# CameronDiao/MolCLR

Measured on AMD Instinct MI355X. Metric: contrastive pre-train molecules/sec at batch 512, 1/2/4/8 MI355X; HBM GB/s on scatter_add, higher is better.
Workload: dtype f32; 1 GPU; c2: GIN 5x300 feat 512, batch 512/GPU, 10-50 atom graphs; model=gin 5x300 feat 512, global_batch=512, per_gpu_batch=512, mean_nodes_per_view=15278, mean_edges_per_view=25094, parallelism=dp1, views=one paired encoder pass, per-view BatchNorm statistics, augment=host: pre-built resident batch pairs

## Files before the change

include/molclr.h:

```cpp
#ifndef MOLCLR_H_
#define MOLCLR_H_

#include <stddef.h>
#include <stdint.h>

#ifdef __cplusplus
extern "C" {
#endif

typedef void* molclr_stream_t;

enum {
  MOLCLR_OK = 0,
  MOLCLR_ERR_ARG = -1,
  MOLCLR_ERR_WORKSPACE = -2,
  MOLCLR_ERR_UNSUPPORTED = -3
};

#define MOLCLR_NUM_ATOM_TYPE 119
#define MOLCLR_NUM_CHIRALITY 3
#define MOLCLR_NUM_BOND_TYPE 5
#define MOLCLR_NUM_BOND_DIR 3
#define MOLCLR_SELF_LOOP_BOND_TYPE 4
#define MOLCLR_ECOUNT_STRIDE 8
#define MOLCLR_NUM_ECOMB 15
#define MOLCLR_SELF_LOOP_ECOMB 12
#define MOLCLR_NBR_SLOTS 4
#define MOLCLR_NBR_OVERFLOW 7
#define MOLCLR_NBR_MAX_NODES (1 << 24)
#define MOLCLR_STATUS_ATOM_RANGE 8

#define MOLCLR_ECOMB(ecode) ((int)((ecode) & 7u) * 3 + (int)((ecode) >> 3))

const char* molclr_version(void);
const char* molclr_last_error(void);

size_t molclr_graph_build_workspace_bytes(int64_t num_nodes, int64_t num_edges);
int molclr_graph_build(const int64_t* edge_index, const int64_t* edge_attr,
                       const int64_t* batch, int64_t num_nodes, int64_t num_edges,
                       int64_t num_graphs, int32_t* rowptr, int32_t* col,
                       uint8_t* ecode, int32_t* rowptr_t, int32_t* col_t,
                       uint32_t* nbr, uint32_t* nbr_t,
                       int32_t* ecount, int32_t* graph_ptr, int32_t* status,
                       void* workspace, size_t workspace_bytes, molclr_stream_t stream);

#define MOLCLR_MAX_SEGMENTS 8
typedef struct molclr_graph_segment {
  const int64_t* edge_index;
  const int64_t* edge_attr;
  const int64_t* batch;
  int64_t num_nodes, num_edges, num_graphs;
} molclr_graph_segment;
int molclr_graph_build_multi(int nseg, const molclr_graph_segment* segs, int32_t* rowptr,
                             int32_t* col, uint8_t* ecode, int32_t* rowptr_t, int32_t* col_t,
                             uint32_t* nbr, uint32_t* nbr_t, int32_t* ecount, int32_t* graph_ptr,
                             int32_t* status, void* workspace, size_t workspace_bytes,
                             molclr_stream_t stream);

typedef struct molclr_stage_source {
  const int64_t *x, *edge_index, *edge_attr, *batch;
  int64_t num_nodes, num_edges;
} molclr_stage_source;
typedef struct molclr_graph_staged_segment {
  const int64_t* edge_index;
  const int64_t* edge_attr;
  const int64_t* batch;
  int64_t node_cap, edge_cap, num_graphs;
} molclr_graph_staged_segment;
int molclr_stage_segments(int nseg, const molclr_stage_source* src,
                          const molclr_graph_staged_segment* dst, int64_t* x_all,
                          int64_t num_nodes_cap, int64_t num_edges_cap, int64_t* counts,
                          molclr_stream_t stream);
int molclr_graph_build_dev(int nseg, const molclr_graph_staged_segment* segs, const int64_t* counts,
                           int64_t num_nodes_cap, int64_t num_edges_cap, int32_t* rowptr,
                           int32_t* col, uint8_t* ecode, int32_t* rowptr_t, int32_t* col_t,
                           uint32_t* nbr, uint32_t* nbr_t, int32_t* ecount, int32_t* graph_ptr,
                           int32_t* status, void* workspace, size_t workspace_bytes,
                           molclr_stream_t stream);

size_t molclr_mask_views_workspace_bytes(int64_t batch_size);
int molclr_mask_views(const int64_t* store_x, const int64_t* store_atom_ptr,
                      const int64_t* store_edge_index, const int64_t* store_edge_attr,
                      const int64_t* store_bond_ptr, int64_t store_mols, int64_t store_edges,
                      const int64_t* mol_ids, int64_t batch_size, uint64_t seed, int view,
                      int64_t* x_out, int64_t* edge_index_out, int64_t* edge_attr_out,
                      int64_t* batch_out, int64_t* ptr_out, int64_t num_nodes, int64_t num_edges,
                      int32_t* status, void* workspace, size_t workspace_bytes,
                      molclr_stream_t stream);

enum { MOLCLR_AUG_SUBGRAPH = 0, MOLCLR_AUG_MIX = 1 };
size_t molclr_aug_views_workspace_bytes(int64_t batch_size, int64_t num_nodes, int64_t num_bonds);
int molclr_aug_views_plan(const int64_t* store_atom_ptr, const int64_t* store_edge_index,
                          const int64_t* store_bond_ptr, int64_t store_mols, int64_t store_edges,
                          const int64_t* mol_ids, int64_t batch_size, uint64_t seed, int view,
                          int mode, int64_t num_nodes, int64_t num_bonds, int64_t* ptr_out,
                          int64_t* num_edges_out, int32_t* status, void* workspace,
                          size_t workspace_bytes, molclr_stream_t stream);
size_t molclr_aug_views_big_workspace_bytes(int64_t big_slots, int64_t big_atoms,
                                            int64_t big_bonds);
int molclr_aug_views_plan_big(const int64_t* store_atom_ptr, const int64_t* store_edge_index,
                              const int64_t* store_bond_ptr, int64_t store_mols,
                              int64_t store_edges, const int64_t* mol_ids, int64_t batch_size,
                              uint64_t seed, int view, int mode, int64_t num_nodes,
                              int64_t num_bonds, int64_t* ptr_out, int64_t* num_edges_out,
                              int32_t* status, void* workspace, size_t workspace_bytes,
                              int64_t big_slots, int64_t big_atoms, int64_t big_bonds,
                              void* big_workspace, size_t big_workspace_bytes,
                              molclr_stream_t stream);
int molclr_aug_views_write(const int64_t* store_x, const int64_t* store_atom_ptr,
                           const int64_t* store_edge_index, const int64_t* store_edge_attr,
                           const int64_t* store_bond_ptr, int64_t store_mols, int64_t store_edges,
                           const int64_t* mol_ids, int64_t batch_size, const int64_t* ptr,
                           int64_t num_nodes, int64_t num_bonds, int64_t num_edges, int64_t* x_out,
                           int64_t* edge_index_out, int64_t* edge_attr_out, int64_t* batch_out,
                           const void* workspace, size_t workspace_bytes, molclr_stream_t stream);

int molclr_atom_embed_fwd(const int64_t* x, const float* X1, const float* X2,
                          float* h, int64_t num_nodes, int64_t dim, int64_t n1,
                          int64_t n2, int32_t* status, molclr_stream_t stream);
size_t molclr_atom_embed_bwd_workspace_bytes(int64_t num_nodes, int64_t dim, int64_t n1,
                                             int64_t n2);
int molclr_atom_embed_bwd(const int64_t* x, const float* dh, float* dX1, float* dX2,
                          int64_t num_nodes, int64_t dim, int64_t n1, int64_t n2, int accumulate,
                          void* workspace, size_t workspace_bytes, molclr_stream_t stream);

#define MOLCLR_MAX_LAYERS 16
int molclr_edge_tables_combine(int layers, const float* const* E1s, const float* const* E2s,
                               float* Ec, int64_t dim, molclr_stream_t stream);

int molclr_gine_aggregate_fwd(const float* x, const int32_t* rowptr, const int32_t* col,
                              const uint8_t* ecode, const uint32_t* nbr, const float* Ec,
                              float* out, int64_t num_nodes, int64_t dim,
                              molclr_stream_t stream);
int64_t molclr_rowmax_layout(int64_t D);
size_t molclr_rowmax_bytes(int64_t N, int64_t D);
int molclr_gine_aggregate_fwd_rowmax(const float* x, const int32_t* rowptr, const int32_t* col,
                                     const uint8_t* ecode, const uint32_t* nbr, const float* Ec,
                                     float* out, int64_t N, int64_t D, float* rowparts,
                                     float* slot, molclr_stream_t stream);
int molclr_gine_aggregate_bn_fwd(const float* z, const float* coeffs, int relu, int nseg,
                                 const int64_t* seg_rows, const int64_t* seg_rows_dev,
                                 const int32_t* rowptr, const int32_t* col, const uint8_t* ecode,
                                 const uint32_t* nbr, const float* Ec, float* out, int64_t N,
                                 int64_t D, float* rowparts, float* slot, molclr_stream_t stream);
size_t molclr_gine_aggregate_bwd_workspace_bytes(int64_t num_nodes, int64_t dim);
int molclr_gine_aggregate_bwd(const float* g, const int32_t* rowptr_t, const int32_t* col_t,
                              const uint32_t* nbr_t, const int32_t* ecount, float* dx, float* dE1, float* dE2,
                              int64_t num_nodes, int64_t dim, int accumulate, void* workspace,
                              size_t workspace_bytes, molclr_stream_t stream);
int molclr_gine_aggregate_bwd_impl(const float* g, const int32_t* rowptr_t, const int32_t* col_t,
                                   const uint32_t* nbr_t, const int32_t* ecount, float* dx,
                                   float* dE1, float* dE2, int64_t num_nodes, int64_t dim,
                                   int accumulate, void* workspace, size_t workspace_bytes,
                                   molclr_stream_t stream, int impl);

int molclr_gcn_aggregate_fwd(const float* xw, const int32_t* rowptr, const int32_t* col,
                             const uint8_t* ecode, const uint32_t* nbr, const float* E1,
                             const float* E2,
                             const float* bias, float* out, int64_t num_nodes,
                             int64_t dim, molclr_stream_t stream);
size_t molclr_gcn_aggregate_bwd_workspace_bytes(int64_t num_nodes, int64_t dim);
int molclr_gcn_aggregate_bwd(const float* g, const int32_t* rowptr_t, const int32_t* col_t,
                             const uint32_t* nbr_t, const int32_t* ecount, float* dxw, float* dE1, float* dE2,
                             float* dbias, int64_t num_nodes, int64_t dim, int accumulate,
                             void* workspace, size_t workspace_bytes, molclr_stream_t stream);
int molclr_gcn_aggregate_fwd_bf16(const uint16_t* xw, const int32_t* rowptr, const int32_t* col,
                                  const uint8_t* ecode, const uint32_t* nbr, const float* E1,
                                  const float* E2, const float* bias, uint16_t* out,
                                  int64_t num_nodes, int64_t dim, molclr_stream_t stream);
int molclr_gcn_aggregate_bwd_bf16(const uint16_t* g, const int32_t* rowptr_t,
                                  const int32_t* col_t, const uint32_t* nbr_t,
                                  const int32_t* ecount, uint16_t* dxw, float* dE1, float* dE2,
                                  float* dbias, int64_t num_nodes, int64_t dim, int accumulate,
                                  void* workspace, size_t workspace_bytes,
                                  molclr_stream_t stream);

enum { MOLCLR_EPI_NONE = 0, MOLCLR_EPI_BIAS = 1, MOLCLR_EPI_BIAS_RELU = 2,
       MOLCLR_EPI_RELU_MASK = 3,
       MOLCLR_EPI_ACCUMULATE = 16  };
size_t molclr_gemm_f32_workspace_bytes(int64_t M, int64_t N, int64_t K);
int molclr_gemm_f32(const float* A, const float* B, float* C, int64_t M, int64_t N,
                    int64_t K, int64_t lda, int64_t ldb, int64_t ldc, int a_kmajor,
                    int b_kmajor, int epilogue_flags, const float* bias, const float* aux,
                    int64_t ldaux, void* workspace, size_t workspace_bytes,
                    molclr_stream_t stream);

int molclr_gemm_f32_impl(const float* A, const float* B, float* C, int64_t M, int64_t N,
                         int64_t K, int64_t lda, int64_t ldb, int64_t ldc, int a_kmajor,
                         int b_kmajor, int epilogue_flags, const float* bias, const float* aux,
                         int64_t ldaux, void* workspace, size_t workspace_bytes,
                         molclr_stream_t stream, int impl);

size_t molclr_bplanes_bytes(int64_t N, int64_t K);
int molclr_bplanes_make(const float* B, int64_t N, int64_t K, int64_t ldb, int b_kmajor,
                        uint16_t* planes, molclr_stream_t stream);
int molclr_bplanes_make_batch(int count, const float* const* B, const int64_t* N,
                              const int64_t* K, const int64_t* ldb, const int* b_kmajor,
                              uint16_t* const* planes, molclr_stream_t stream);
int molclr_gemm_f32_bplanes(const float* A, const uint16_t* planes, float* C, int64_t M,
                            int64_t N, int64_t K, int64_t lda, int64_t ldc, int a_kmajor,
                            int epilogue_flags, const float* bias, const float* aux,
                            int64_t ldaux, void* workspace, size_t workspace_bytes,
                            molclr_stream_t stream);
int molclr_gemm_f32_bplanes_tile(const float* A, const uint16_t* planes, float* C, int64_t M,
                                 int64_t N, int64_t K, int64_t lda, int64_t ldc, int a_kmajor,
                                 int epilogue_flags, const float* bias, const float* aux,
                                 int64_t ldaux, void* workspace, size_t workspace_bytes,
                                 molclr_stream_t stream, int tile);

size_t molclr_linear_wgrad_workspace_bytes(int64_t rows, int64_t n_out, int64_t n_in);
int molclr_linear_wgrad(const float* dy, const float* x, float* dW, float* db, int64_t rows,
// ... 134 lines not shown
                                int accumulate, void* workspace, size_t workspace_bytes,
                                molclr_stream_t stream);
int molclr_batchnorm_seg_bwd_frozen(const void* dy, const void* z, const float* gamma,
                                    const float* beta, const float* save_mean,
                                    const float* save_invstd, void* dz, float* dgamma,
                                    float* dbeta, int nseg, const int64_t* seg_rows, int64_t dim,
                                    int dtype, int relu, int accumulate, void* workspace,
                                    size_t workspace_bytes, molclr_stream_t stream);
int molclr_batchnorm_seg_bwd_frozen_dev(const void* dy, const void* z, const float* gamma,
                                        const float* beta, const float* save_mean,
                                        const float* save_invstd, void* dz, float* dgamma,
                                        float* dbeta, int nseg, const int64_t* seg_rows_dev,
                                        int64_t rows_cap, int64_t dim, int dtype, int relu,
                                        int accumulate, float* rowmax, float* slot,
                                        void* workspace, size_t workspace_bytes,
                                        molclr_stream_t stream);
int molclr_batchnorm_seg_bwd_frozen_max(const float* dy, const float* z, const float* gamma,
                                        const float* beta, const float* save_mean,
                                        const float* save_invstd, float* dz, float* dgamma,
                                        float* dbeta, int nseg, const int64_t* seg_rows,
                                        int64_t dim, int relu, int accumulate, float* rowmax,
                                        float* slot, void* workspace, size_t workspace_bytes,
                                        molclr_stream_t stream);

int molclr_segment_pool_fwd(const float* h, const int32_t* graph_ptr, float* out,
                            int64_t num_graphs, int64_t dim, int mode,
                            molclr_stream_t stream);
int molclr_segment_pool_bwd(const float* dout, const int32_t* graph_ptr, float* dh,
                            int64_t num_nodes, int64_t num_graphs, int64_t dim, int mode,
                            molclr_stream_t stream);
int molclr_segment_max_fwd(const void* h, const int32_t* graph_ptr, float* out, int32_t* argmax,
                           int64_t num_graphs, int64_t dim, int dtype, molclr_stream_t stream);
int molclr_segment_max_bwd(const float* dout, const int32_t* argmax, void* dh, int64_t num_nodes,
                           int64_t num_graphs, int64_t dim, int dtype, molclr_stream_t stream);

int molclr_l2norm_fwd(const float* z, float* y, float* norm, int64_t rows, int64_t dim,
                      double eps, molclr_stream_t stream);
int molclr_l2norm_bwd(const float* dy, const float* y, const float* norm, float* dz,
                      int64_t rows, int64_t dim, double eps, molclr_stream_t stream);

int molclr_ntxent_prep(const float* r, float* rhat, float* norm, int64_t n, int64_t C,
                       int cosine, molclr_stream_t stream);
int molclr_ntxent_prep_bwd(const float* drhat, const float* rhat, const float* norm,
                           float* dr, int64_t n, int64_t C, int cosine,
                           molclr_stream_t stream);
int molclr_ntxent_prep_pair(const float* z, float* y, float* rhat, float* n1, float* n2,
                            int64_t batch_local, int64_t C, double eps, int cosine,
                            molclr_stream_t stream);
int molclr_ntxent_prep_pair_bwd(const float* drhat, const float* rhat, const float* n2,
                                const float* y, const float* n1, float* dz, int64_t batch_local,
                                int64_t C, double eps, int cosine, molclr_stream_t stream);
size_t molclr_ntxent_workspace_bytes(int64_t nrows, int64_t ncols, int64_t C);
int molclr_ntxent_fwd(const float* rhat_rows, const int32_t* row_gidx, const float* rhat_cols,
                      int64_t nrows, int64_t ncols, int64_t C, int64_t batch_size,
                      double temperature, float* lse_rows, float* loss_rows,
                      void* workspace, size_t workspace_bytes, molclr_stream_t stream);
int molclr_ntxent_bwd(const float* rhat_rows, const int32_t* row_gidx, const float* rhat_cols,
                      const float* lse_cols, const float* grad_loss, int64_t nrows,
                      int64_t ncols, int64_t C, int64_t batch_size, double temperature,
                      float* drhat_rows, void* workspace, size_t workspace_bytes,
                      molclr_stream_t stream);
size_t molclr_ntxent_sim_bytes(int64_t nrows, int64_t ncols, int64_t C, int impl);
int molclr_ntxent_fwd_impl(const float* rhat_rows, const int32_t* row_gidx,
                           const float* rhat_cols, int64_t nrows, int64_t ncols, int64_t C,
                           int64_t batch_size, double temperature, float* lse_rows,
                           float* loss_rows, float* sim, void* workspace, size_t workspace_bytes,
                           molclr_stream_t stream, int impl);
int molclr_ntxent_bwd_impl(const float* rhat_rows, const int32_t* row_gidx,
                           const float* rhat_cols, const float* lse_cols, const float* grad_loss,
                           int64_t nrows, int64_t ncols, int64_t C, int64_t batch_size,
                           double temperature, const float* sim, float* drhat_rows,
                           void* workspace, size_t workspace_bytes, molclr_stream_t stream,
                           int impl);
int molclr_sum_f32(const float* x, float* out, int64_t n, molclr_stream_t stream);

int molclr_adam_step(float* param, const float* grad, float* exp_avg, float* exp_avg_sq,
                     int64_t n, const float* lr, int32_t* step, double beta1, double beta2,
                     double eps, double weight_decay, molclr_stream_t stream);
int molclr_adam_step_ex(float* param, const float* grad, float* exp_avg, float* exp_avg_sq,
                        int64_t n, const float* lr, int32_t* step, double beta1, double beta2,
                        double eps, double weight_decay, int tick, molclr_stream_t stream);
int molclr_step_tail(int32_t* step, const float* loss_src, float* loss_dst,
                     const int32_t* status_src, int32_t* status_acc, molclr_stream_t stream);

enum {
  MOLCLR_MODE_EVAL = 0,
  MOLCLR_MODE_TRAIN = 1,
  MOLCLR_MODE_FROZEN_BN = 2
};
typedef struct molclr_gin_encoder {
  int32_t num_layer;
  int32_t training;
  int64_t dim;
  int64_t n_atom;
  int64_t n_chiral;
  double momentum, eps;
  const float* x_embedding1;
  const float* x_embedding2;
  const float* mlp0_weight[MOLCLR_MAX_LAYERS];
  const float* mlp0_bias[MOLCLR_MAX_LAYERS];
  const float* mlp2_weight[MOLCLR_MAX_LAYERS];
  const float* mlp2_bias[MOLCLR_MAX_LAYERS];
  const float* edge_embedding1[MOLCLR_MAX_LAYERS];
  const float* edge_embedding2[MOLCLR_MAX_LAYERS];
  const float* bn_weight[MOLCLR_MAX_LAYERS];
  const float* bn_bias[MOLCLR_MAX_LAYERS];
  float* bn_running_mean[MOLCLR_MAX_LAYERS];
  float* bn_running_var[MOLCLR_MAX_LAYERS];
  int64_t* bn_num_batches_tracked[MOLCLR_MAX_LAYERS];
  const uint16_t* mlp0_planes[MOLCLR_MAX_LAYERS];
  const uint16_t* mlp0_planes_t[MOLCLR_MAX_LAYERS];
  const uint16_t* mlp2_planes[MOLCLR_MAX_LAYERS];
  const uint16_t* mlp2_planes_t[MOLCLR_MAX_LAYERS];
  int32_t dtype;
  int32_t fp32_gemm;
  int32_t* status;
  double drop_ratio;
  int64_t* drop_state;
} molclr_gin_encoder;

typedef struct molclr_gin_encoder_grads {
  float* x_embedding1;
  float* x_embedding2;
  float* mlp0_weight[MOLCLR_MAX_LAYERS];
  float* mlp0_bias[MOLCLR_MAX_LAYERS];
  float* mlp2_weight[MOLCLR_MAX_LAYERS];
  float* mlp2_bias[MOLCLR_MAX_LAYERS];
  float* edge_embedding1[MOLCLR_MAX_LAYERS];
  float* edge_embedding2[MOLCLR_MAX_LAYERS];
  float* bn_weight[MOLCLR_MAX_LAYERS];
  float* bn_bias[MOLCLR_MAX_LAYERS];
  void* layer_done[MOLCLR_MAX_LAYERS];
  void* embed_done;
} molclr_gin_encoder_grads;

typedef struct molclr_device_graph {
  int64_t num_nodes, num_edges, num_graphs;
  const int32_t *rowptr, *col, *rowptr_t, *col_t, *ecount, *graph_ptr;
  const uint8_t* ecode;
  const uint32_t *nbr, *nbr_t;
  int32_t num_segments;
  int64_t segment_nodes[MOLCLR_MAX_SEGMENTS];
  const int64_t* segment_nodes_dev;
} molclr_device_graph;

size_t molclr_gin_encoder_arena_bytes(int num_layer, int64_t num_nodes, int64_t dim, int dtype);
size_t molclr_gin_encoder_workspace_bytes(int num_layer, int64_t num_nodes, int64_t dim,
                                          int dtype);
int molclr_gin_encoder_fwd(const molclr_gin_encoder* enc, const int64_t* x,
                           const molclr_device_graph* graph, void* h_out, void* arena,
                           size_t arena_bytes, void* workspace, size_t workspace_bytes,
                           molclr_stream_t stream);
int molclr_gin_encoder_bwd(const molclr_gin_encoder* enc, const molclr_gin_encoder_grads* grads,
                           const int64_t* x, const molclr_device_graph* graph,
                           const void* dh_out, const void* arena, size_t arena_bytes,
                           void* workspace, size_t workspace_bytes, molclr_stream_t stream);

typedef struct molclr_gcn_encoder {
  int32_t num_layer;
  int32_t training;
  int64_t dim;
  int64_t n_atom;
  int64_t n_chiral;
  double momentum, eps;
  const float* x_embedding1;
  const float* x_embedding2;
// ... 244 lines not shown
```

molclr_amd/_lib.py:

```python
from __future__ import annotations

import ctypes
import os
from ctypes import POINTER, c_char_p, c_double, c_int, c_int64, c_size_t, c_uint64, c_void_p
from pathlib import Path

import torch

LIB_PATH = Path(os.environ.get("MOLCLR_LIB", Path(__file__).resolve().parent / "libmolclr_hip.so"))

_P = c_void_p
_I64 = c_int64

SIGNATURES = {
    "molclr_version": (c_char_p, []),
    "molclr_last_error": (c_char_p, []),
    "molclr_graph_build_workspace_bytes": (c_size_t, [_I64, _I64]),
    "molclr_graph_build": (c_int, [_P, _P, _P, _I64, _I64, _I64, _P, _P, _P, _P, _P, _P, _P, _P,
                                   _P, _P, _P, c_size_t, _P]),
    "molclr_graph_build_multi": (c_int, [c_int, _P, _P, _P, _P, _P, _P, _P, _P, _P, _P, _P, _P,
                                         c_size_t, _P]),
    "molclr_stage_segments": (c_int, [c_int, _P, _P, _P, _I64, _I64, _P, _P]),
    "molclr_graph_build_dev": (c_int, [c_int, _P, _P, _I64, _I64, _P, _P, _P, _P, _P, _P, _P, _P,
                                       _P, _P, _P, c_size_t, _P]),
    "molclr_mask_views_workspace_bytes": (c_size_t, [_I64]),
    "molclr_mask_views": (c_int, [_P, _P, _P, _P, _P, _I64, _I64, _P, _I64, c_uint64, c_int, _P, _P,
                                  _P, _P, _P, _I64, _I64, _P, _P, c_size_t, _P]),
    "molclr_atom_embed_fwd": (c_int, [_P, _P, _P, _P, _I64, _I64, _I64, _I64, _P, _P]),
    "molclr_atom_embed_bwd_workspace_bytes": (c_size_t, [_I64, _I64, _I64, _I64]),
    "molclr_atom_embed_bwd": (c_int, [_P, _P, _P, _P, _I64, _I64, _I64, _I64, c_int, _P, c_size_t,
                                      _P]),
    "molclr_edge_tables_combine": (c_int, [c_int, _P, _P, _P, _I64, _P]),
    "molclr_gine_aggregate_fwd": (c_int, [_P, _P, _P, _P, _P, _P, _P, _I64, _I64, _P]),
    "molclr_rowmax_layout": (_I64, [_I64]),
    "molclr_rowmax_bytes": (c_size_t, [_I64, _I64]),
    "molclr_gine_aggregate_fwd_rowmax": (c_int, [_P, _P, _P, _P, _P, _P, _P, _I64, _I64, _P, _P,
                                                 _P]),
    "molclr_gine_aggregate_bn_fwd": (c_int, [_P, _P, c_int, c_int, _P, _P, _P, _P, _P, _P, _P, _P,
                                             _I64, _I64, _P, _P, _P]),
    "molclr_gine_aggregate_bn_fwd_bf16": (c_int, [_P, _P, c_int, c_int, _P, _P, _P, _P, _P, _P, _P,
                                                  _P, _I64, _I64, _P]),
    "molclr_batchnorm_seg_coeffs": (c_int, [_P, _P, _P, _P, _P, _P, _P, _P, _P, c_int, _P, _I64,
                                            c_int, c_double, c_double, c_int, _P, c_size_t, _P]),
    "molclr_batchnorm_seg_coeffs_dev": (c_int, [_P, _P, _P, _P, _P, _P, _P, _P, _P, c_int, _P, _I64,
                                                _I64, c_int, c_double, c_double, c_int, _P,
                                                c_size_t, _P]),
    "molclr_gine_aggregate_bwd_workspace_bytes": (c_size_t, [_I64, _I64]),
    "molclr_gine_aggregate_bwd": (c_int, [_P, _P, _P, _P, _P, _P, _P, _P, _I64, _I64, c_int, _P,
                                          c_size_t, _P]),
    "molclr_gine_aggregate_bwd_impl": (c_int, [_P, _P, _P, _P, _P, _P, _P, _P, _I64, _I64, c_int,
                                               _P, c_size_t, _P, c_int]),
    "molclr_gcn_aggregate_fwd": (c_int, [_P, _P, _P, _P, _P, _P, _P, _P, _P, _I64, _I64, _P]),
    "molclr_gcn_aggregate_bwd_workspace_bytes": (c_size_t, [_I64, _I64]),
    "molclr_gcn_aggregate_bwd": (c_int, [_P, _P, _P, _P, _P, _P, _P, _P, _P, _I64, _I64, c_int,
                                         _P, c_size_t, _P]),
    "molclr_gcn_aggregate_fwd_bf16": (c_int, [_P, _P, _P, _P, _P, _P, _P, _P, _P, _I64, _I64, _P]),
    "molclr_gcn_aggregate_bwd_bf16": (c_int, [_P, _P, _P, _P, _P, _P, _P, _P, _P, _I64, _I64,
                                              c_int, _P, c_size_t, _P]),
    "molclr_gemm_f32_workspace_bytes": (c_size_t, [_I64, _I64, _I64]),
    "molclr_gemm_f32": (c_int, [_P, _P, _P, _I64, _I64, _I64, _I64, _I64, _I64, c_int, c_int, c_int,
                                _P, _P, _I64, _P, c_size_t, _P]),
    "molclr_gemm_f32_impl": (c_int, [_P, _P, _P, _I64, _I64, _I64, _I64, _I64, _I64, c_int, c_int,
                                     c_int, _P, _P, _I64, _P, c_size_t, _P, c_int]),
    "molclr_bplanes_bytes": (c_size_t, [_I64, _I64]),
    "molclr_bplanes_make": (c_int, [_P, _I64, _I64, _I64, c_int, _P, _P]),
    "molclr_bplanes_make_batch": (c_int, [c_int, _P, _P, _P, _P, _P, _P, _P]),
    "molclr_gemm_f32_bplanes": (c_int, [_P, _P, _P, _I64, _I64, _I64, _I64, _I64, c_int, c_int, _P,
                                        _P, _I64, _P, c_size_t, _P]),
    "molclr_gemm_f32_bplanes_tile": (c_int, [_P, _P, _P, _I64, _I64, _I64, _I64, _I64, c_int,
                                             c_int, _P, _P, _I64, _P, c_size_t, _P, c_int]),
    "molclr_linear_wgrad_workspace_bytes": (c_size_t, [_I64, _I64, _I64]),
    "molclr_linear_wgrad": (c_int, [_P, _P, _P, _P, _I64, _I64, _I64, _I64, _I64, c_int, _P, c_size_t,
                                    _P]),
    "molclr_linear_wgrad_groups": (c_int, [_P, _P, _P, _P, _I64, _I64, _I64, _I64, _I64, c_int, _P,
                                           c_size_t, _P, c_int]),
    "molclr_absmax_f32": (c_int, [_P, _I64, _I64, _I64, _P, c_int, _P]),
    "molclr_hplanes_bytes": (c_size_t, [_I64, _I64]),
    "molclr_hplanes_make_batch": (c_int, [c_int, _P, _P, _P, _P, _P, _P, _P]),
    "molclr_absmax_rows_f32": (c_int, [_P, _I64, _I64, _I64, _P, _P, c_int, _P]),
    "molclr_bn_row_parts": (c_int, [_I64]),
    "molclr_batchnorm_seg_bwd_max": (c_int, [_P, _P, _P, _P, _P, _P, _P, _P, _P, c_int, _P, _I64,
                                             c_int, c_int, _P, _P, _P, c_size_t, _P]),
    "molclr_gemm_row_parts": (_I64, [_I64]),
    "molclr_gemm_f32_bplanes_max": (c_int, [_P, _P, _P, _I64, _I64, _I64, _I64, _I64, c_int, _P,
                                            _P, _I64, _P, _P, _P, _P, _P, c_size_t, _P]),
    "molclr_gemm_f32_h3": (c_int, [_P, _P, c_int, _P, _P, _I64, _I64, _I64, _I64, _I64, c_int, _P,
                                   _P, _I64, _P, _P, _P, _P, _P]),
    "molclr_gemm_f32_h3_bits": (c_int, [_P, _P, c_int, _P, _P, _I64, _I64, _I64, _I64, _I64, c_int,
                                        _P, _P, _I64, _P, _P, _P, _P, _P, _P]),
    "molclr_gemm_f32_h3_impl": (c_int, [_P, _P, c_int, _P, _P, _I64, _I64, _I64, _I64, _I64, c_int,
                                        _P, _P, _I64, _P, _P, _P, _P, _P, _P, c_int]),
    "molclr_linear_wgrad_h3_groups": (c_int, [_P, _P, _P, _P, _P, _P, _I64, _I64, _I64, _I64, _I64,
                                              c_int, _P, c_size_t, _P, c_int]),
    "molclr_linear_wgrad_h3": (c_int, [_P, _P, _P, _P, _P, _P, _I64, _I64, _I64, _I64, _I64, c_int,
                                       _P, c_size_t, _P]),
    "molclr_colsum_f32_workspace_bytes": (c_size_t, [_I64, _I64]),
    "molclr_colsum_f32": (c_int, [_P, _P, _I64, _I64, _I64, c_int, _P, c_size_t, _P]),
    "molclr_batchnorm_workspace_bytes": (c_size_t, [_I64, _I64]),
    "molclr_batchnorm_fwd": (c_int, [_P, _P, _P, _P, _P, _P, _P, _P, _P, _I64, _I64, c_double,
                                     c_double, c_int, c_int, _P, c_size_t, _P]),
    "molclr_batchnorm_bwd": (c_int, [_P, _P, _P, _P, _P, _P, _P, _P, _P, _I64, _I64, c_int, c_int,
                                     _P, c_size_t, _P]),
    "molclr_batchnorm_bwd_frozen": (c_int, [_P, _P, _P, _P, _P, _P, _P, _P, _P, _I64, _I64, c_int,
                                            c_int, _P, c_size_t, _P]),
    "molclr_batchnorm_seg_bwd_frozen": (c_int, [_P, _P, _P, _P, _P, _P, _P, _P, _P, c_int, _P, _I64,
                                                c_int, c_int, c_int, _P, c_size_t, _P]),
    "molclr_batchnorm_seg_bwd_frozen_dev": (c_int, [_P, _P, _P, _P, _P, _P, _P, _P, _P, c_int, _P,
                                                    _I64, _I64, c_int, c_int, c_int, _P, _P, _P,
                                                    c_size_t, _P]),
    "molclr_batchnorm_seg_bwd_frozen_max": (c_int, [_P, _P, _P, _P, _P, _P, _P, _P, _P, c_int, _P,
                                                    _I64, c_int, c_int, _P, _P, _P, c_size_t, _P]),
    "molclr_batchnorm_seg_workspace_bytes": (c_size_t, [c_int, _P, _I64]),
    "molclr_batchnorm_seg_fwd": (c_int, [_P, _P, _P, _P, _P, _P, _P, _P, _P, c_int, _P, _I64, c_int,
                                         c_double, c_double, c_int, c_int, _P, c_size_t, _P]),
    "molclr_batchnorm_seg_bwd": (c_int, [_P, _P, _P, _P, _P, _P, _P, _P, _P, c_int, _P, _I64, c_int,
                                         c_int, c_int, _P, c_size_t, _P]),
    "molclr_batchnorm_seg_dev_workspace_bytes": (c_size_t, [c_int, _I64, _I64]),
    "molclr_batchnorm_seg_fwd_dev": (c_int, [_P, _P, _P, _P, _P, _P, _P, _P, _P, c_int, _P, _I64,
                                             _I64, c_int, c_double, c_double, c_int, c_int, _P,
                                             c_size_t, _P]),
    "molclr_batchnorm_seg_bwd_dev": (c_int, [_P, _P, _P, _P, _P, _P, _P, _P, _P, c_int, _P, _I64,
                                             _I64, c_int, c_int, c_int, _P, _P, _P, c_size_t, _P]),
    "molclr_segment_pool_fwd": (c_int, [_P, _P, _P, _I64, _I64, c_int, _P]),
    "molclr_segment_pool_bwd": (c_int, [_P, _P, _P, _I64, _I64, _I64, c_int, _P]),
    "molclr_l2norm_fwd": (c_int, [_P, _P, _P, _I64, _I64, c_double, _P]),
    "molclr_l2norm_bwd": (c_int, [_P, _P, _P, _P, _I64, _I64, c_double, _P]),
    "molclr_ntxent_prep": (c_int, [_P, _P, _P, _I64, _I64, c_int, _P]),
    "molclr_ntxent_prep_bwd": (c_int, [_P, _P, _P, _P, _I64, _I64, c_int, _P]),
    "molclr_ntxent_prep_pair": (c_int, [_P, _P, _P, _P, _P, _I64, _I64, c_double, c_int, _P]),
    "molclr_ntxent_prep_pair_bwd": (c_int, [_P, _P, _P, _P, _P, _P, _I64, _I64, c_double, c_int,
                                            _P]),
    "molclr_ntxent_workspace_bytes": (c_size_t, [_I64, _I64, _I64]),
    "molclr_ntxent_fwd": (c_int, [_P, _P, _P, _I64, _I64, _I64, _I64, c_double, _P, _P, _P,
                                  c_size_t, _P]),
    "molclr_ntxent_bwd": (c_int, [_P, _P, _P, _P, _P, _I64, _I64, _I64, _I64, c_double, _P, _P,
                                  c_size_t, _P]),
    "molclr_ntxent_sim_bytes": (c_size_t, [_I64, _I64, _I64, c_int]),
    "molclr_ntxent_fwd_impl": (c_int, [_P, _P, _P, _I64, _I64, _I64, _I64, c_double, _P, _P,
                                       _P, _P, c_size_t, _P, c_int]),
    "molclr_ntxent_bwd_impl": (c_int, [_P, _P, _P, _P, _P, _I64, _I64, _I64, _I64, c_double, _P,
                                       _P, _P, c_size_t, _P, c_int]),
    "molclr_sum_f32": (c_int, [_P, _P, _I64, _P]),
    "molclr_linear_wgrad_h3_pair_workspace_bytes": (c_size_t, [_I64, _I64, _I64, _I64, _I64]),
    "molclr_linear_wgrad_h3_pair": (c_int, [_P, _P, _P, _P, _P, _P, _I64, _I64, _I64, _I64,
                                            _P, _P, _P, _P, _P, _P, _I64, _I64, _I64, _I64,
                                            _I64, c_int, _P, c_size_t, _P]),
    "molclr_adam_step": (c_int, [_P, _P, _P, _P, _I64, _P, _P, c_double, c_double, c_double,
                                 c_double, _P]),
    "molclr_adam_step_ex": (c_int, [_P, _P, _P, _P, _I64, _P, _P, c_double, c_double, c_double,
                                    c_double, c_int, _P]),
    "molclr_step_tail": (c_int, [_P, _P, _P, _P, _P, _P]),
    "molclr_gin_encoder_arena_bytes": (c_size_t, [c_int, _I64, _I64, c_int]),
    "molclr_gin_encoder_workspace_bytes": (c_size_t, [c_int, _I64, _I64, c_int]),
    "molclr_gin_encoder_fwd": (c_int, [_P, _P, _P, _P, _P, c_size_t, _P, c_size_t, _P]),
    "molclr_gin_encoder_bwd": (c_int, [_P, _P, _P, _P, _P, _P, c_size_t, _P, c_size_t, _P]),
    "molclr_gcn_encoder_arena_bytes": (c_size_t, [c_int, _I64, _I64]),
    "molclr_gcn_encoder_workspace_bytes": (c_size_t, [c_int, _I64, _I64]),
    "molclr_gcn_encoder_arena_bytes_dtype": (c_size_t, [c_int, _I64, _I64, c_int]),
    "molclr_gcn_encoder_workspace_bytes_dtype": (c_size_t, [c_int, _I64, _I64, c_int]),
    "molclr_gcn_encoder_fwd": (c_int, [_P, _P, _P, _P, _P, c_size_t, _P, c_size_t, _P]),
    "molclr_gcn_encoder_bwd": (c_int, [_P, _P, _P, _P, _P, _P, c_size_t, _P, c_size_t, _P]),
    "molclr_dropout_next_key": (c_int, [_P, _P, _P]),
    "molclr_dropout_mask": (c_int, [_P, c_int, c_double, _P, _I64, _I64, _P]),
    "molclr_aug_views_workspace_bytes": (c_size_t, [_I64, _I64, _I64]),
    "molclr_aug_views_plan": (c_int, [_P, _P, _P, _I64, _I64, _P, _I64, ctypes.c_uint64, c_int,
                                      c_int, _I64, _I64, _P, _P, _P, _P, c_size_t, _P]),
    "molclr_aug_views_big_workspace_bytes": (c_size_t, [_I64, _I64, _I64]),
    "molclr_aug_views_plan_big": (c_int, [_P, _P, _P, _I64, _I64, _P, _I64, ctypes.c_uint64,
                                          c_int, c_int, _I64, _I64, _P, _P, _P, _P, c_size_t,
                                          _I64, _I64, _I64, _P, c_size_t, _P]),
    "molclr_aug_views_write": (c_int, [_P, _P, _P, _P, _P, _I64, _I64, _P, _I64, _P, _I64, _I64,
                                       _I64, _P, _P, _P, _P, _P, c_size_t, _P]),
    "molclr_atom_embed_fwd_bf16": (c_int, [_P, _P, _P, _P, _I64, _I64, _I64, _I64, _P, _P]),
    "molclr_atom_embed_bwd_bf16": (c_int, [_P, _P, _P, _P, _I64, _I64, _I64, _I64, c_int, _P,
                                           c_size_t, _P]),
    "molclr_gine_aggregate_fwd_bf16": (c_int, [_P, _P, _P, _P, _P, _P, _P, _I64, _I64, _P]),
    "molclr_gine_aggregate_bwd_bf16": (c_int, [_P, _P, _P, _P, _P, _P, _P, _P, _I64, _I64, c_int,
                                               _P, c_size_t, _P]),
    "molclr_segment_max_fwd": (c_int, [_P, _P, _P, _P, _I64, _I64, c_int, _P]),
    "molclr_segment_max_bwd": (c_int, [_P, _P, _P, _I64, _I64, _I64, c_int, _P]),
    "molclr_segment_pool_fwd_bf16": (c_int, [_P, _P, _P, _I64, _I64, c_int, _P]),
    "molclr_segment_pool_bwd_bf16": (c_int, [_P, _P, _P, _I64, _I64, _I64, c_int, _P]),
    "molclr_gemm_bf16": (c_int, [_P, _P, _P, _I64, _I64, _I64, _I64, _I64, c_int, _P, _P, _I64,
                                 _P]),
    "molclr_gemm_bf16_bits": (c_int, [_P, _P, _P, _I64, _I64, _I64, _I64, _I64, c_int, _P, _P, _P,
                                      _P]),
    "molclr_gemm_bf16_impl": (c_int, [_P, _P, _P, _I64, _I64, _I64, _I64, _I64, c_int, _P, _P,
                                      _I64, _P, c_int]),
    "molclr_linear_wgrad_bf16_workspace_bytes": (c_size_t, [_I64, _I64, _I64]),
    "molclr_linear_wgrad_bf16_impl": (c_int, [_P, _P, _P, _P, _I64, _I64, _I64, _I64, _I64, c_int,
                                              _P, c_size_t, _P, c_int]),
    "molclr_linear_wgrad_bf16": (c_int, [_P, _P, _P, _P, _I64, _I64, _I64, _I64, _I64, c_int, _P,
                                         c_size_t, _P]),
    "molclr_task_head_workspace_bytes": (c_size_t, [_P]),
    "molclr_task_head_fwd": (c_int, [_P, _P, c_size_t, _P]),
    "molclr_task_head_bwd": (c_int, [_P, _P, _P, c_size_t, _P]),
    "molclr_motif_pool_workspace_bytes": (c_size_t, [_I64, _I64, _I64]),
    "molclr_motif_pool_fwd": (c_int, [_P, _P, _P, _P, _P, _P, _I64, _I64, _I64, _I64, _P, _P, _P,
                                      _P]),
    "molclr_motif_pool_bwd": (c_int, [_P, _P, _P, _P, _P, _P, _P, _P, _P, _P, _I64, _I64, _I64, _I64,
                                      _P, _P, _P, _P, c_int, c_int, c_int, _P, c_size_t, _P]),
    "molclr_motif_pool_cap_workspace_bytes": (c_size_t, [_I64, _I64, _I64]),
    "molclr_motif_pool_fwd_cap": (c_int, [_P, _P, _P, _P, _P, _P, _I64, _I64, _I64, _I64, _P, _P,
                                          _P, _P]),
    "molclr_motif_pool_bwd_cap": (c_int, [_P, _P, _P, _P, _P, _P, _P, _P, _P, _P, _I64, _I64, _I64,
                                          _I64, _P, _P, _P, _P, c_int, c_int, c_int, _P, c_size_t,
                                          _P]),
    "molclr_stage_motif": (c_int, [_P, _P, _I64, _I64, _I64, _P, _P, _P, _P, _P, _P]),
    "molclr_stage_task": (c_int, [_P, _P, _P, _I64, _I64, _P, _P, _P, _I64, _I64, c_int, _P]),
    "molclr_task_step_tail": (c_int, [_P, _P, _P, _P, _P, _P, _P]),
    "molclr_eval_tail": (c_int, [_P, _P, _I64, _I64, _I64, _P, _P, _P, _I64, _P, _P, _P, _P, _P]),
    "molclr_collate_task_workspace_bytes": (c_size_t, [_I64]),
    "molclr_collate_task": (c_int, [_P, _P, _P, _P, _P, _I64, _I64, _P, _I64, _P, _I64, c_int, _P,
                                    _P, _P, _P, _P, _P, _I64, _I64, _P, _P, c_size_t, _P]),
    "molclr_stage_task_ids": (c_int, [_P, _P, _P, _P, _P, _I64, _I64, _P, _I64, _P, _I64, c_int,
                                      _I64, _I64, _P, _P, _I64, _I64, _P, _P, _P, _P, c_size_t,
                                      _P]),
    "molclr_motif_items_workspace_bytes": (c_size_t, [_I64]),
    "molclr_motif_items": (c_int, [_P, _P, _I64, _P, _I64, _I64, _P, _P, _P, _P, c_size_t, _P]),
    "molclr_stage_motif_ids_workspace_bytes": (c_size_t, [_I64, _I64]),
    "molclr_stage_motif_ids": (c_int, [_P, _P, _I64, _P, _I64, _I64, _I64, _P, _P, _P, _P, _P, _P,
                                       c_size_t, _P]),
    "molclr_topk_dot_workspace_bytes": (c_size_t, [_I64, _I64, _I64, c_int]),
    "molclr_topk_dot": (c_int, [_P, _I64, _P, _I64, c_int, _I64, _I64, _I64, c_int, _P, _I64, _P,
                                _P, _P, c_size_t, _P]),
    "molclr_ktimer_start": (c_int, [c_int]),
    "molclr_ktimer_read": (c_int, [c_int, _P, _P]),
    "molclr_ktimer_stop": (c_int, []),
}

EPI_NONE, EPI_BIAS, EPI_BIAS_RELU, EPI_RELU_MASK = 0, 1, 2, 3
EPI_ACCUMULATE = 16
NUM_ECOMB = 15
MAX_LAYERS = 16
# ... 165 lines not shown
```

molclr_amd/csrc/aggregate.hip:

```cpp
#include "common.h"

#include <stdlib.h>

namespace {

constexpr int kT = 256;

template <typename St, int U = 1>
__global__ void k_atom_embed_fwd(const int64_t* __restrict__ x, const float4* __restrict__ X1,
                                 const float4* __restrict__ X2, typename St::T* __restrict__ h,
                                 int64_t N, int d4, int64_t n1, int64_t n2,
                                 int32_t* __restrict__ status) {
  int64_t t = (int64_t)blockIdx.x * blockDim.x + threadIdx.x;
  if (t >= N * d4 / U) return;
  const int64_t u0 = t * U;
  int64_t i = N * d4 < (1ll << 32) ? (int64_t)((uint32_t)u0 / (uint32_t)d4) : u0 / d4;
  int c = (int)(u0 - i * d4);
  const int64_t a = x[2 * i], b = x[2 * i + 1];
  float4 v[U];
  if (a < 0 || a >= n1 || b < 0 || b >= n2) {
    const float q = __builtin_nanf("");
#pragma unroll
    for (int j = 0; j < U; ++j) v[j] = make_float4(q, q, q, q);
    if (c == 0 && status != nullptr) atomicOr(status, MOLCLR_STATUS_ATOM_RANGE);
  } else {
#pragma unroll
    for (int j = 0; j < U; ++j) v[j] = f4add(X1[a * d4 + c + j], X2[b * d4 + c + j]);
  }
  if constexpr (U == 2) St::st2(h, t, v[0], v[1]);
  else St::st(h, t, v[0]);
}

constexpr int kEmbBlock = 256;
constexpr int kEmbChunk = 128;

__device__ __forceinline__ int emb_key(const int64_t* __restrict__ x, int64_t item, int64_t N,
                                       int64_t n1, int64_t n2) {
  if (item < N) {
    const int64_t a = x[2 * item];
    return (int)(a < 0 ? 0 : (a >= n1 ? n1 - 1 : a));
  }
  const int64_t b = x[2 * (item - N) + 1];
  return (int)(n1 + (b < 0 ? 0 : (b >= n2 ? n2 - 1 : b)));
}

__global__ __launch_bounds__(kEmbBlock) void k_emb_hist(const int64_t* __restrict__ x, int64_t N,
                                                        int64_t n1, int64_t n2,
                                                        int32_t* __restrict__ hist) {
  extern __shared__ int32_t h[];
  const int nk = (int)(n1 + n2);
  for (int k = threadIdx.x; k < nk; k += kEmbBlock) h[k] = 0;
  __syncthreads();
  const int64_t item = (int64_t)blockIdx.x * kEmbBlock + threadIdx.x;
  if (item < 2 * N) atomicAdd(&h[emb_key(x, item, N, n1, n2)], 1);
  __syncthreads();
  for (int k = threadIdx.x; k < nk; k += kEmbBlock) hist[(int64_t)k * gridDim.x + blockIdx.x] = h[k];
}

__global__ __launch_bounds__(64) void k_emb_keyscan(int32_t* __restrict__ hist, int nblk,
                                                    int32_t* __restrict__ total) {
  const int64_t k = blockIdx.x;
  const int lane = threadIdx.x;
  int32_t* row = hist + k * nblk;
  int32_t carry = 0;
  for (int base = 0; base < nblk; base += 64) {
    const int b = base + lane;
    const int32_t v = b < nblk ? row[b] : 0;
    int32_t incl = v;
#pragma unroll
    for (int o = 1; o < 64; o <<= 1) {
      const int32_t u = __shfl_up(incl, o, 64);
      if (lane >= o) incl += u;
    }
    if (b < nblk) row[b] = carry + incl - v;
    carry += __shfl(incl, 63, 64);
  }
  if (lane == 0) total[k] = carry;
}

__global__ __launch_bounds__(1024) void k_emb_plan(const int32_t* __restrict__ total, int nk,
                                                   int32_t* __restrict__ kstart,
                                                   int32_t* __restrict__ cbeg,
                                                   int32_t* __restrict__ cend,
                                                   int32_t* __restrict__ kchunk0,
                                                   int32_t* __restrict__ nchunks, int max_chunks) {
  __shared__ int32_t tot[1024], ks[1025], kc[1025];
  const int t = threadIdx.x;
  tot[t] = t < nk ? total[t] : 0;
  __syncthreads();
  if (t == 0) {
    int32_t run = 0, ch = 0;
    for (int k = 0; k < nk; ++k) {
      ks[k] = run;
      kc[k] = ch;
      run += tot[k];
      ch += (tot[k] + kEmbChunk - 1) / kEmbChunk;
    }
    ks[nk] = run;
    kc[nk] = ch;
    *nchunks = ch;
  }
  __syncthreads();
  for (int k = t; k <= nk; k += 1024) {
    kstart[k] = ks[k];
    kchunk0[k] = kc[k];
  }
  const int nch = kc[nk];
  for (int c = t; c < max_chunks; c += 1024) {
    if (c >= nch) break;
    int lo = 0, hi = nk - 1;
    while (lo < hi) {
      const int mid = (lo + hi + 1) >> 1;
      if (kc[mid] <= c) lo = mid;
// ... 49 lines not shown
  for (; i + 4 <= end; i += 4) {
    float4 v[4];
#pragma unroll
    for (int u = 0; u < 4; ++u) v[u] = St::ld(dh, (int64_t)perm[i + u] * d4 + c);
#pragma unroll
    for (int u = 0; u < 4; ++u) acc = f4add(acc, v[u]);
  }
  for (; i < end; ++i) acc = f4add(acc, St::ld(dh, (int64_t)perm[i] * d4 + c));
  double* o = csum + ch * 4 * d4 + 4 * c;
  o[0] = acc.x;
  o[1] = acc.y;
  o[2] = acc.z;
  o[3] = acc.w;
}

constexpr int kEmbFinW = 8;
__global__ __launch_bounds__(64 * kEmbFinW) void k_emb_finish(
    const double* __restrict__ csum, const int32_t* __restrict__ kchunk0, int64_t n1, int64_t n2,
    int64_t D, float* __restrict__ dX1, float* __restrict__ dX2, int accumulate) {
  __shared__ double red[kEmbFinW][64];
  const int lane = threadIdx.x & 63, w = threadIdx.x >> 6;
  const int64_t k = blockIdx.x;
  const int64_t col = (int64_t)blockIdx.y * 64 + lane;
  double acc = 0.0;
  if (col < D) {
    int32_t ch = kchunk0[k] + w;
    const int32_t ce = kchunk0[k + 1];
    for (; ch + 7 * kEmbFinW < ce; ch += 8 * kEmbFinW) {
      double v[8];
#pragma unroll
      for (int u = 0; u < 8; ++u) v[u] = csum[(int64_t)(ch + u * kEmbFinW) * D + col];
#pragma unroll
      for (int u = 0; u < 8; ++u) acc += v[u];
    }
    for (; ch < ce; ch += kEmbFinW) acc += csum[(int64_t)ch * D + col];
  }
  red[w][lane] = acc;
  __syncthreads();
  if (w != 0 || col >= D) return;
  double t = red[0][lane];
#pragma unroll
  for (int q = 1; q < kEmbFinW; ++q) t += red[q][lane];
  float* o = k < n1 ? dX1 + k * D + col : dX2 + (k - n1) * D + col;
  *o = accumulate ? *o + (float)t : (float)t;
}

__global__ __launch_bounds__(1024) void k_reduce_partials_split(
    const double* __restrict__ partial, int64_t P, int64_t rows, int64_t D, int64_t split,
    float* __restrict__ outA, float* __restrict__ outB, int accumulate) {
  constexpr int EL = 16, LANES = 64;
  __shared__ double red[LANES][EL];
  const int cl = threadIdx.x % EL, rl = threadIdx.x / EL;
  const int64_t t = (int64_t)blockIdx.x * EL + cl;
  const int64_t n = rows * D;
  double a0 = 0.0, a1 = 0.0, a2 = 0.0, a3 = 0.0;
  if (t < n) {
    int64_t p = rl;
    for (; p + 3 * LANES < P; p += 4 * LANES) {
      a0 += partial[p * n + t];
      a1 += partial[(p + LANES) * n + t];
      a2 += partial[(p + 2 * LANES) * n + t];
      a3 += partial[(p + 3 * LANES) * n + t];
    }
    for (; p < P; p += LANES) a0 += partial[p * n + t];
  }
  double acc = (a0 + a1) + (a2 + a3);
  red[rl][cl] = acc;
  __syncthreads();
#pragma unroll
  for (int stride = LANES / 2; stride > 0; stride >>= 1) {
    if (rl < stride) red[rl][cl] = acc = acc + red[rl + stride][cl];
    __syncthreads();
  }
  if (rl != 0 || t >= n) return;
  int64_t r = t / D;
  float* o = r < split ? (outA ? outA + t : nullptr) : (outB ? outB + (t - split * D) : nullptr);
  if (o) *o = accumulate ? *o + (float)acc : (float)acc;
}

struct TablePtrs {
  const float* e1[MOLCLR_MAX_LAYERS];
  const float* e2[MOLCLR_MAX_LAYERS];
};
__global__ void k_edge_tables_combine(TablePtrs p, float* __restrict__ Ec, int layers, int64_t D,
                                      float* __restrict__ zero, int64_t n_zero) {
  const int64_t per = (int64_t)MOLCLR_NUM_ECOMB * D;
  int64_t t = (int64_t)blockIdx.x * blockDim.x + threadIdx.x;
  if (t < n_zero) zero[t] = 0.f;
  if (t >= layers * per) return;
  const int l = (int)(t / per);
  const int64_t rc = t - l * per;
  const int r = (int)(rc / D);
  const int64_t c = rc - (int64_t)r * D;
  Ec[t] = p.e1[l][(r / 3) * D + c] + p.e2[l][(r % 3) * D + c];
}

__device__ __forceinline__ uint32_t nbr_degree(uint32_t w0) { return w0 >> 29; }
__device__ __forceinline__ int32_t nbr_node(uint32_t w) { return (int32_t)(w & 0xFFFFFFu); }
__device__ __forceinline__ int nbr_ecomb(uint32_t w) { return (int)((w >> 24) & 15u); }

__device__ __forceinline__ float4 gine_msg(const float4* __restrict__ x, const float4* __restrict__ Ec,
                                           uint32_t w, int d4, int c) {
  return f4add(x[(int64_t)nbr_node(w) * d4 + c], Ec[nbr_ecomb(w) * d4 + c]);
}

struct NoSrcArgs {};
template <typename DR>
struct BnSrcArgsT {
  const float4* scale;
  const float4* shift;
  int relu;
  Segs sg;
  DR drop;
};
typedef BnSrcArgsT<NoDrop> BnSrcArgs;

template <typename St, typename DR>
__device__ __forceinline__ float4 bn_src_unit(float4 v, float4 sc, float4 sh, bool relu,
                                              const Drop<DR>& drop, int64_t j, int c4) {
  float4 o = make_float4(bn_apply1(v.x, sc.x, sh.x), bn_apply1(v.y, sc.y, sh.y),
                         bn_apply1(v.z, sc.z, sh.z), bn_apply1(v.w, sc.w, sh.w));
  if (relu) o = make_float4(fmaxf(o.x, 0.f), fmaxf(o.y, 0.f), fmaxf(o.z, 0.f), fmaxf(o.w, 0.f));
  if constexpr (DR::kOn) o = drop(o, j, c4);
  if constexpr (St::kBytes == 2) {
    const uint32_t lo = f32x2_to_bf16x2(o.x, o.y), hi = f32x2_to_bf16x2(o.z, o.w);
    o = make_float4(bf16_to_f32(lo & 0xFFFFu), bf16_to_f32(lo >> 16), bf16_to_f32(hi & 0xFFFFu),
                    bf16_to_f32(hi >> 16));
  }
  return o;
}

template <typename St, typename SA>
struct AggSrc {
  __device__ __forceinline__ AggSrc(const SA&, int64_t, int, int) {}
  __device__ __forceinline__ float4 operator()(const typename St::T* __restrict__ x, int64_t unit,
                                               int64_t) const {
    return St::ld(x, unit);
  }
};
template <typename St, typename DR>
struct AggSrc<St, BnSrcArgsT<DR>> {
  float4 sc, sh;
  bool relu, pad;
  int c;
  Drop<DR> drop;
  __device__ __forceinline__ AggSrc(const BnSrcArgsT<DR>& a, int64_t i, int c_, int d4)
      : c(c_), drop(a.drop) {
    const int s = seg_of_row(a.sg, i);
    pad = s < 0;
    relu = a.relu != 0;
    sc = pad ? f4zero() : a.scale[s * d4 + c];
    sh = pad ? f4zero() : a.shift[s * d4 + c];
  }
  __device__ __forceinline__ float4 operator()(const typename St::T* __restrict__ x, int64_t unit,
                                               int64_t j) const {
    if (pad) return f4zero();
    return bn_src_unit<St, DR>(St::ld(x, unit), sc, sh, relu, drop, j, c);
  }
};

template <typename St, bool NT = false, typename SA = NoSrcArgs>
__device__ __forceinline__ float4 gine_agg_elem(
    const typename St::T* __restrict__ x, const int32_t* __restrict__ rowptr,
    const int32_t* __restrict__ col, const uint8_t* __restrict__ ecode,
    const uint4* __restrict__ nbr, const float4* __restrict__ Ec, typename St::T* __restrict__ out,
    int64_t t, int64_t i, int c, int d4, const SA& sa) {
  const AggSrc<St, SA> src(sa, i, c, d4);
  auto X = [&](int64_t j) { return src(x, j * d4 + c, j); };
  auto msg = [&](uint32_t w) {
    return f4add(X((int64_t)nbr_node(w)), Ec[nbr_ecomb(w) * d4 + c]);
  };
  const uint4 s = nbr[i];
  const float4 self = src(x, t, i);
  const float4 es = Ec[MOLCLR_SELF_LOOP_ECOMB * d4 + c];
  const uint32_t deg = nbr_degree(s.x);
  float4 acc = f4zero();
  if (deg <= MOLCLR_NBR_SLOTS) {
// ... 558 lines not shown

template <typename St>
int emb_bwd(const int64_t* x, const typename St::T* dh, float* dX1, float* dX2, int64_t N,
            int64_t D, int64_t n1, int64_t n2, int accumulate, void* workspace,
            size_t workspace_bytes, hipStream_t s) {
  const int64_t nk = n1 + n2;
  const EmbWs e = emb_ws(workspace, workspace_bytes, N, D, n1, n2);
  const int64_t d4 = D / 4;
  if (N > 0) {
    hipLaunchKernelGGL(k_emb_hist, dim3((unsigned)e.nblk), dim3(kEmbBlock), nk * sizeof(int32_t), s,
                       x, N, n1, n2, e.hist);
  } else {
    (void)molclr::zero_async(e.hist, (size_t)e.nblk * nk * sizeof(int32_t), s);
  }
  hipLaunchKernelGGL(k_emb_keyscan, dim3((unsigned)nk), dim3(64), 0, s, e.hist, (int)e.nblk,
                     e.total);
  hipLaunchKernelGGL(k_emb_plan, dim3(1), dim3(1024), 0, s, static_cast<const int32_t*>(e.total),
                     (int)nk, e.kstart, e.cbeg, e.cend, e.kchunk0, e.nchunks, (int)e.max_chunks);
  if (N > 0) {
    hipLaunchKernelGGL(k_emb_scatter, dim3((unsigned)e.nblk), dim3(kEmbBlock), 0, s, x, N, n1, n2,
                       static_cast<const int32_t*>(e.hist), static_cast<const int32_t*>(e.kstart),
                       e.perm);
    hipLaunchKernelGGL(k_emb_chunk_sum<St>, dim3((unsigned)e.max_chunks,
                                                 (unsigned)molclr::ceil_div(d4, 64)),
                       dim3(64), 0, s, dh, static_cast<const int32_t*>(e.perm),
                       static_cast<const int32_t*>(e.cbeg), static_cast<const int32_t*>(e.cend),
                       static_cast<const int32_t*>(e.nchunks), d4, e.csum);
  }
  hipLaunchKernelGGL(k_emb_finish, dim3((unsigned)nk, (unsigned)molclr::ceil_div(D, 64)),
                     dim3(64 * kEmbFinW), 0, s,
                     static_cast<const double*>(e.csum), static_cast<const int32_t*>(e.kchunk0), n1,
                     n2, D, dX1, dX2, accumulate);
  MOLCLR_LAUNCHED();
  return MOLCLR_OK;
}
}

MOLCLR_API size_t molclr_atom_embed_bwd_workspace_bytes(int64_t N, int64_t D, int64_t n1,
                                                        int64_t n2) {
  const int64_t nk = n1 + n2;
  const int64_t nblk = molclr::ceil_div(2 * N > 0 ? 2 * N : 1, (int64_t)kEmbBlock);
  const int64_t max_chunks = molclr::ceil_div(2 * N, (int64_t)kEmbChunk) + nk;
  return (size_t)(nblk * nk + nk + 2 * (nk + 1) + 2 * max_chunks + 1 + 2 * N) * sizeof(int32_t) +
         (size_t)max_chunks * D * sizeof(double) + 10 * 256;
}

MOLCLR_API int molclr_atom_embed_bwd(const int64_t* x, const float* dh, float* dX1, float* dX2,
                                     int64_t N, int64_t D, int64_t n1, int64_t n2, int accumulate,
                                     void* workspace, size_t workspace_bytes,
                                     molclr_stream_t stream) {
  MOLCLR_REQUIRE(D > 0 && D % 4 == 0 && n1 > 0 && n2 > 0 && N >= 0,
                 "atom_embed_bwd: bad sizes (dim a multiple of 4)");
  MOLCLR_REQUIRE(n1 + n2 <= 1024, "atom_embed_bwd: tables too large");
  MOLCLR_REQUIRE(2 * N < (1ll << 31), "atom_embed_bwd: too many nodes");
  MOLCLR_REQUIRE_WS(workspace_bytes, molclr_atom_embed_bwd_workspace_bytes(N, D, n1, n2));
  return emb_bwd<StF32>(x, dh, dX1, dX2, N, D, n1, n2, accumulate, workspace, workspace_bytes,
                        molclr::as_stream(stream));
}

MOLCLR_API int molclr_edge_tables_combine(int layers, const float* const* E1s,
                                          const float* const* E2s, float* Ec, int64_t D,
                                          molclr_stream_t stream) {
  return molclr::edge_tables_combine_zero(layers, E1s, E2s, Ec, D, nullptr, 0, stream);
}

int molclr::edge_tables_combine_zero(int layers, const float* const* E1s, const float* const* E2s,
                                     float* Ec, int64_t D, float* zero, int64_t n_zero,
                                     molclr_stream_t stream) {
  MOLCLR_REQUIRE(layers >= 0 && layers <= MOLCLR_MAX_LAYERS && D > 0,
                 "edge_tables_combine: %d layers (max %d), dim %lld", layers, MOLCLR_MAX_LAYERS,
                 (long long)D);
  if (layers == 0) return MOLCLR_OK;
  MOLCLR_REQUIRE(E1s && E2s && Ec, "edge_tables_combine: null pointer");
  TablePtrs p{};
  for (int l = 0; l < layers; ++l) {
    MOLCLR_REQUIRE(E1s[l] && E2s[l], "edge_tables_combine: null table of layer %d", l);
    p.e1[l] = E1s[l];
    p.e2[l] = E2s[l];
  }
  const int64_t n = (int64_t)layers * MOLCLR_NUM_ECOMB * D;
  const int64_t work = n > n_zero ? n : n_zero;
  hipLaunchKernelGGL(k_edge_tables_combine, dim3(molclr::ceil_div(work, kT)), dim3(kT), 0,
                     molclr::as_stream(stream), p, Ec, layers, D, zero, n_zero);
  MOLCLR_LAUNCHED();
  return MOLCLR_OK;
}

static bool agg_nt() {
  static const bool on = molclr::env_is("MOLCLR_AGG_NT", '1');
  return on;
}

MOLCLR_API int molclr_gine_aggregate_fwd(const float* x, const int32_t* rowptr,
                                         const int32_t* col, const uint8_t* ecode,
                                         const uint32_t* nbr, const float* Ec, float* out,
                                         int64_t N, int64_t D, molclr_stream_t stream) {
  MOLCLR_REQUIRE(D > 0 && D % 4 == 0, "gine_aggregate_fwd: dim %lld must be a multiple of 4",
                 (long long)D);
  if (N == 0) return MOLCLR_OK;
  MOLCLR_REQUIRE(x && rowptr && nbr && Ec && out, "gine_aggregate_fwd: null pointer");
  int d4 = (int)(D / 4);
  molclr::launch_timed(molclr::kTimeGineAgg, agg_nt() ? k_gine_agg_fwd<StF32, false, true>
                                                      : k_gine_agg_fwd<StF32, false, false>,
                       dim3(molclr::ceil_div(N * d4, kT)), dim3(kT), 0, molclr::as_stream(stream),
                       x, rowptr, col, ecode, (const uint4*)nbr, (const float4*)Ec, out, N, d4,
                       nullptr, 0, nullptr, NoSrcArgs{});
  MOLCLR_LAUNCHED();
  return MOLCLR_OK;
}

MOLCLR_API int64_t molclr_rowmax_layout(int64_t D) {
  const int64_t d4 = D / 4;
  return d4 >= 64 ? -d4 : (int64_t)molclr_bn_row_parts(D);
}
MOLCLR_API size_t molclr_rowmax_bytes(int64_t N, int64_t D) {
  const int64_t code = molclr_rowmax_layout(D);
  return code < 0 ? (size_t)((N * (D / 4) + 63) / 64) * 2 * sizeof(float)
                  : (size_t)code * N * sizeof(float);
}

MOLCLR_API int molclr_gine_aggregate_fwd_rowmax(const float* x, const int32_t* rowptr,
                                                const int32_t* col, const uint8_t* ecode,
                                                const uint32_t* nbr, const float* Ec, float* out,
                                                int64_t N, int64_t D, float* rowparts, float* slot,
                                                molclr_stream_t stream) {
  MOLCLR_REQUIRE(D > 0 && D % 4 == 0, "gine_aggregate_fwd_rowmax: dim %lld must be a multiple of 4",
                 (long long)D);
  MOLCLR_REQUIRE(N < (1ll << 31), "gine_aggregate_fwd_rowmax: too many rows");
  if (N == 0) return MOLCLR_OK;
  MOLCLR_REQUIRE(x && rowptr && nbr && Ec && out && rowparts,
                 "gine_aggregate_fwd_rowmax: null pointer");
  const int d4 = (int)(D / 4);
  static_assert(kT % 64 == 0, "row parts follow the waves");
  molclr::launch_timed(molclr::kTimeGineAgg, agg_nt() ? k_gine_agg_fwd<StF32, true, true>
                                                      : k_gine_agg_fwd<StF32, true, false>,
                       dim3(molclr::ceil_div(N * d4, kT)), dim3(kT), 0, molclr::as_stream(stream),
                       x, rowptr, col, ecode, (const uint4*)nbr, (const float4*)Ec, out, N, d4,
                       rowparts, (int)molclr_rowmax_layout(D), slot, NoSrcArgs{});
  MOLCLR_LAUNCHED();
  return MOLCLR_OK;
}

MOLCLR_API size_t molclr_gine_aggregate_bwd_workspace_bytes(int64_t N, int64_t D) {
  if (!molclr::band_dim_ok(D)) return 0;
  return (size_t)ecount_parts(N, molclr::make_band(D).band) * 8 * D * sizeof(double) + 256;
}

static bool agg_bwd_fused() {
  static const bool on = !molclr::env_is("MOLCLR_AGG_BWD_FUSED", '0');
  return on;
}

MOLCLR_API int molclr_gine_aggregate_bwd_impl(const float* g, const int32_t* rowptr_t,
                                              const int32_t* col_t, const uint32_t* nbr_t,
                                              const int32_t* ecount, float* dx, float* dE1,
                                              float* dE2, int64_t N, int64_t D, int accumulate,
                                              void* workspace, size_t workspace_bytes,
                                              molclr_stream_t stream, int impl) {
  MOLCLR_REQUIRE(molclr::band_dim_ok(D),
                 "gine_aggregate_bwd: dim %lld must be a multiple of 4 in [4, %lld]", (long long)D,
                 (long long)molclr::kBandMaxDim);
  MOLCLR_REQUIRE(impl >= -1 && impl <= 1, "gine_aggregate_bwd: impl %d (-1, 0 or 1)", impl);
  hipStream_t s = molclr::as_stream(stream);
  int d4 = (int)(D / 4);
  const bool fusable = dx && (dE1 || dE2) && N > 0;
  if (fusable && (impl < 0 ? agg_bwd_fused() : impl == 1)) {
// ... 382 lines not shown
```

molclr_amd/csrc/encoder.hip:

```cpp
#include "common.h"

#include <stdlib.h>

namespace {

bool agg_bn() {
  static const bool on = !molclr::env_is("MOLCLR_AGG_BN", '0');
  return on;
}

struct ArenaLayout {
  size_t agg[MOLCLR_MAX_LAYERS], a1[MOLCLR_MAX_LAYERS], z[MOLCLR_MAX_LAYERS],
      h[MOLCLR_MAX_LAYERS], mean[MOLCLR_MAX_LAYERS], invstd[MOLCLR_MAX_LAYERS],
      coef[MOLCLR_MAX_LAYERS];
  size_t bits[MOLCLR_MAX_LAYERS];
  size_t h0, ec, smax, bmax, dropkey, total;
  ArenaLayout(int L, int64_t N, int64_t D, size_t es) {
    size_t used = 0;
    auto off = [&](size_t bytes) {
      const size_t o = used;
      used += (bytes + 255) / 256 * 256;
      return o;
    };
    for (int l = 0; l < L; ++l) {
      agg[l] = off(N * D * es);
      a1[l] = off(N * 2 * D * es);
      z[l] = off(N * D * es);
      h[l] = agg_bn() ? 0 : off(N * D * es);
      mean[l] = off(MOLCLR_MAX_SEGMENTS * D * sizeof(float));
      invstd[l] = off(MOLCLR_MAX_SEGMENTS * D * sizeof(float));
      coef[l] = off(2 * MOLCLR_MAX_SEGMENTS * D * sizeof(float));
      bits[l] = off((size_t)N * ((2 * D + 31) / 32) * sizeof(uint32_t));
    }
    h0 = off(N * D * es);
    ec = off((size_t)L * MOLCLR_NUM_ECOMB * D * sizeof(float));
    smax = off((size_t)MOLCLR_MAX_LAYERS * 2 * kMaxSlotFloats * sizeof(float));
    bmax = off((size_t)MOLCLR_MAX_LAYERS * 2 * kMaxSlotFloats * sizeof(float));
    dropkey = off(2 * sizeof(int64_t));
    total = used;
  }
};

size_t elem_bytes(int dtype) { return dtype == MOLCLR_DTYPE_BF16 ? 2 : 4; }

size_t kernels_ws(int64_t N, int64_t D) {
  size_t m = 0;
  auto mx = [&](size_t v) { m = v > m ? v : m; };
  mx(molclr_gemm_f32_workspace_bytes(2 * D, D, N));
  mx(molclr_gemm_f32_workspace_bytes(D, 2 * D, N));
  mx(molclr_gemm_f32_workspace_bytes(N, 2 * D, D));
  mx(molclr_gemm_f32_workspace_bytes(N, D, 2 * D));
  mx(molclr_colsum_f32_workspace_bytes(N, 2 * D));
  mx(molclr_linear_wgrad_workspace_bytes(N, D, 2 * D));
  mx(molclr_linear_wgrad_workspace_bytes(N, 2 * D, D));
  if (N >= 1024 && D % 4 == 0) mx(molclr_linear_wgrad_h3_pair_workspace_bytes(N, D, 2 * D, 2 * D, D));
  mx(molclr_linear_wgrad_bf16_workspace_bytes(N, D, 2 * D));
  mx(molclr_linear_wgrad_bf16_workspace_bytes(N, 2 * D, D));
  mx(molclr_batchnorm_ws_bound(N, D));
  mx(molclr_gine_aggregate_bwd_workspace_bytes(N, D));
  mx(molclr_atom_embed_bwd_workspace_bytes(N, D, MOLCLR_NUM_ATOM_TYPE, MOLCLR_NUM_CHIRALITY));
  return m;
}

size_t scratch_bytes(int64_t N, int64_t D, size_t es) { return ((size_t)N * D * 3 + (size_t)N * 2 * D) * es; }

template <typename E>
int bn_batch_stats(const E* e) { return e->training == MOLCLR_MODE_TRAIN; }

int check_drop(const char* who, double drop_ratio, const int64_t* drop_state, int training) {
  MOLCLR_REQUIRE(training == MOLCLR_MODE_EVAL || training == MOLCLR_MODE_TRAIN ||
                     training == MOLCLR_MODE_FROZEN_BN,
                 "%s: training %d (MOLCLR_MODE_*)", who, training);
  MOLCLR_REQUIRE(drop_ratio >= 0.0 && drop_ratio < 1.0, "%s: drop_ratio %g outside [0, 1)", who,
                 drop_ratio);
  MOLCLR_REQUIRE(!(training && drop_ratio > 0.0) || drop_state,
                 "%s: training with dropout needs drop_state", who);
  return MOLCLR_OK;
}

int check_encoder(const molclr_gin_encoder* e, const molclr_device_graph* g) {
  MOLCLR_REQUIRE(e && g, "gin_encoder: null encoder / graph");
  MOLCLR_TRY_RC(check_drop("gin_encoder", e->drop_ratio, e->drop_state, e->training));
  MOLCLR_REQUIRE(e->num_layer >= 1 && e->num_layer <= MOLCLR_MAX_LAYERS,
                 "gin_encoder: num_layer %d", e->num_layer);
  MOLCLR_REQUIRE(e->dim > 0 && e->dim % 4 == 0, "gin_encoder: dim %lld", (long long)e->dim);
  MOLCLR_REQUIRE(e->dtype == MOLCLR_DTYPE_F32 || (e->dtype == MOLCLR_DTYPE_BF16 && e->dim % 8 == 0),
                 "gin_encoder: dtype %d (bf16 needs dim %% 8 == 0)", e->dtype);
  MOLCLR_REQUIRE(e->n_atom == MOLCLR_NUM_ATOM_TYPE && e->n_chiral == MOLCLR_NUM_CHIRALITY,
                 "gin_encoder: embedding tables must be [%d,D] and [%d,D]",
                 MOLCLR_NUM_ATOM_TYPE, MOLCLR_NUM_CHIRALITY);
// ... 82 lines not shown
    if (!on) return nullptr;
    cur = make_drop_args(key, p, l);
    return &cur;
  }
};
int open_drop(const CallDrop& d, int64_t* state, molclr_stream_t stream) {
  if (!d.on) return MOLCLR_OK;
  return molclr_dropout_next_key(state, const_cast<int64_t*>(d.key), stream);
}

#define MOLCLR_TRY(expr)      \
  do {                        \
    int rc_ = (expr);         \
    if (rc_) return rc_;      \
  } while (0)

int record_done(void* ev, molclr_stream_t stream) {
  if (ev && hipEventRecord(static_cast<hipEvent_t>(ev), molclr::as_stream(stream)) != hipSuccess) {
    molclr::set_error("encoder_bwd: hipEventRecord failed");
    return MOLCLR_ERR_ARG;
  }
  return MOLCLR_OK;
}

}

MOLCLR_API size_t molclr_gin_encoder_arena_bytes(int L, int64_t N, int64_t D, int dtype) {
  if (L < 1 || L > MOLCLR_MAX_LAYERS) return 0;
  return ArenaLayout(L, N, D, elem_bytes(dtype)).total;
}

constexpr size_t kSlotBytes = MOLCLR_MAX_LAYERS * 2 * kMaxSlotFloats * sizeof(float);
size_t rowmax_first_bytes(int64_t N, int64_t D) {
  const size_t dz = (size_t)molclr_bn_row_parts(D) * N * sizeof(float);
  const size_t agg = molclr_rowmax_bytes(N, D);
  return molclr::align_up(dz > agg ? dz : agg, 256);
}
size_t rowmax_bytes(int64_t N, int64_t D) {
  return molclr::align_up(
      rowmax_first_bytes(N, D) + (size_t)molclr_gemm_row_parts(2 * D) * N * sizeof(float), 256);
}

MOLCLR_API size_t molclr_gin_encoder_workspace_bytes(int L, int64_t N, int64_t D, int dtype) {
  (void)L;
  return molclr::align_up(scratch_bytes(N, D, elem_bytes(dtype)), 256) + kSlotBytes +
         rowmax_bytes(N, D) + kernels_ws(N, D) + 256;
}

MOLCLR_API int molclr_gin_encoder_fwd(const molclr_gin_encoder* e, const int64_t* x,
                                      const molclr_device_graph* g, void* h_out, void* arena,
                                      size_t arena_bytes, void* workspace, size_t workspace_bytes,
                                      molclr_stream_t stream) {
  MOLCLR_TRY(check_encoder(e, g));
  const int L = e->num_layer;
  const int64_t N = g->num_nodes, D = e->dim;
  if (N == 0) return MOLCLR_OK;
  SegRows seg;
  MOLCLR_TRY(graph_segments(g, &g->num_nodes, seg));
  MOLCLR_REQUIRE(x && h_out && arena, "gin_encoder_fwd: null pointer");
  const bool bf = e->dtype == MOLCLR_DTYPE_BF16;
  const size_t es = elem_bytes(e->dtype);
  const ArenaLayout lay(L, N, D, es);
  MOLCLR_REQUIRE_WS(arena_bytes, lay.total);
  MOLCLR_REQUIRE_WS(workspace_bytes, molclr_gin_encoder_workspace_bytes(L, N, D, e->dtype));
  char* A = (char*)arena;
  auto F = [&](size_t off) { return (float*)(A + off); };
  auto H = [&](size_t off) { return (uint16_t*)(A + off); };
  float* ragg = (float*)((char*)workspace + molclr::align_up(scratch_bytes(N, D, es), 256) +
                         kSlotBytes);
  float* ra1 = (float*)((char*)ragg + rowmax_first_bytes(N, D));
  void* kws = (char*)ragg + rowmax_bytes(N, D);
  const size_t kws_bytes = kernels_ws(N, D);
  const bool h3 = !bf && e->fp32_gemm != 0;
  const bool h3f = h3 && (e->fp32_gemm & 2);
  float* fmax = F(lay.smax);

  const bool fused = agg_bn();
  CallDrop drop(e->training, e->drop_ratio, A + lay.dropkey);
  MOLCLR_TRY(open_drop(drop, e->drop_state, stream));
  void* h = A + lay.h0;
  if (bf)
    MOLCLR_TRY(molclr_atom_embed_fwd_bf16(x, e->x_embedding1, e->x_embedding2, (uint16_t*)h, N, D,
                                          e->n_atom, e->n_chiral, e->status, stream));
  else
    MOLCLR_TRY(molclr_atom_embed_fwd(x, e->x_embedding1, e->x_embedding2, (float*)h, N, D,
                                     e->n_atom, e->n_chiral, e->status, stream));
  float* Ec = F(lay.ec);
  const int64_t nz = h3 ? (int64_t)(lay.bmax - lay.smax) / 4 + (int64_t)L * 2 * kMaxSlotFloats : 0;
  MOLCLR_TRY(molclr::edge_tables_combine_zero(L, e->edge_embedding1, e->edge_embedding2, Ec, D,
                                              h3 ? fmax : nullptr, nz, stream));
  for (int l = 0; l < L; ++l) {
    const bool last = l == L - 1;
    const bool bn_src = fused && l > 0;
    const bool bn_next = fused && !last;
    void* y = last ? h_out : bn_next ? nullptr : A + lay.h[l];
    const float* Ecl = Ec + (size_t)l * MOLCLR_NUM_ECOMB * D;
    const void* zp = bn_src ? A + lay.z[l - 1] : nullptr;
    const float* cp = bn_src ? F(lay.coef[l - 1]) : nullptr;
    if (bf) {
      uint16_t *agg = H(lay.agg[l]), *a1 = H(lay.a1[l]), *z = H(lay.z[l]);
      if (bn_src && drop.on)
        MOLCLR_TRY(molclr::gine_aggregate_bn_fwd_drop(zp, cp, 1, seg.n, seg.rows, seg.dev,
                                                      g->rowptr, g->col, g->ecode, g->nbr, Ecl,
                                                      agg, N, D, MOLCLR_DTYPE_BF16, nullptr,
                                                      nullptr, *drop.at(l - 1),
                                                      molclr::as_stream(stream)));
      else if (bn_src)
        MOLCLR_TRY(molclr_gine_aggregate_bn_fwd_bf16((const uint16_t*)zp, cp, 1, seg.n, seg.rows,
                                                     seg.dev, g->rowptr, g->col, g->ecode, g->nbr,
                                                     Ecl, agg, N, D, stream));
      else
        MOLCLR_TRY(molclr_gine_aggregate_fwd_bf16((const uint16_t*)h, g->rowptr, g->col, g->ecode,
                                                  g->nbr, Ecl, agg, N, D, stream));
      if (D % 64 == 0)
        MOLCLR_TRY(molclr_gemm_bf16_bits(agg, e->mlp0_planes[l], a1, N, 2 * D, D, D, 2 * D,
                                         MOLCLR_EPI_BIAS_RELU, e->mlp0_bias[l],
                                         (uint32_t*)(A + lay.bits[l]), nullptr, stream));
      else
        MOLCLR_TRY(molclr_gemm_bf16(agg, e->mlp0_planes[l], a1, N, 2 * D, D, D, 2 * D,
                                    MOLCLR_EPI_BIAS_RELU, e->mlp0_bias[l], nullptr, 0, stream));
      MOLCLR_TRY(molclr_gemm_bf16(a1, e->mlp2_planes[l], z, N, D, 2 * D, 2 * D, D,
                                  MOLCLR_EPI_BIAS, e->mlp2_bias[l], nullptr, 0, stream));
      if (bn_next)
        MOLCLR_TRY(seg_bn_coeffs(seg, z, e->bn_weight[l], e->bn_bias[l], e->bn_running_mean[l],
                                 e->bn_running_var[l], e->bn_num_batches_tracked[l],
                                 F(lay.mean[l]), F(lay.invstd[l]), F(lay.coef[l]), D,
                                 MOLCLR_DTYPE_BF16, e->momentum, e->eps, bn_batch_stats(e), kws,
                                 kws_bytes, stream));
      else
        MOLCLR_TRY(seg_bn_fwd(seg, z, e->bn_weight[l], e->bn_bias[l], e->bn_running_mean[l],
                              e->bn_running_var[l], e->bn_num_batches_tracked[l], y,
                              F(lay.mean[l]), F(lay.invstd[l]), D, MOLCLR_DTYPE_BF16, e->momentum,
                              e->eps, bn_batch_stats(e), last ? 0 : 1, drop.at(l), kws, kws_bytes,
                              stream));
    } else {
      float *agg = F(lay.agg[l]), *a1 = F(lay.a1[l]), *z = F(lay.z[l]);
      float* sl = fmax + 2 * l * kMaxSlotFloats;
      if (bn_src && drop.on)
        MOLCLR_TRY(molclr::gine_aggregate_bn_fwd_drop(zp, cp, 1, seg.n, seg.rows, seg.dev,
                                                      g->rowptr, g->col, g->ecode, g->nbr, Ecl,
                                                      agg, N, D, MOLCLR_DTYPE_F32,
                                                      h3f ? ragg : nullptr, nullptr,
                                                      *drop.at(l - 1), molclr::as_stream(stream)));
      else if (bn_src)
        MOLCLR_TRY(molclr_gine_aggregate_bn_fwd((const float*)zp, cp, 1, seg.n, seg.rows, seg.dev,
                                                g->rowptr, g->col, g->ecode, g->nbr, Ecl, agg, N,
                                                D, h3f ? ragg : nullptr, nullptr, stream));
      else if (h3f)
        MOLCLR_TRY(molclr_gine_aggregate_fwd_rowmax((const float*)h, g->rowptr, g->col, g->ecode,
                                                    g->nbr, Ecl, agg, N, D, ragg, nullptr,
                                                    stream));
      else
        MOLCLR_TRY(molclr_gine_aggregate_fwd((const float*)h, g->rowptr, g->col, g->ecode, g->nbr,
                                             Ecl, agg, N, D, stream));
      if (h3f) {
        const uint16_t* p0 = e->mlp0_planes[l];
        const uint16_t* p2 = e->mlp2_planes[l];
        MOLCLR_TRY(molclr_gemm_f32_h3_bits(agg, ragg, (int)molclr_rowmax_layout(D), p0, a1, N,
                                           2 * D, D, D, 2 * D, MOLCLR_EPI_BIAS_RELU,
                                           e->mlp0_bias[l], nullptr, 0, nullptr,
                                           sl + kMaxSlotFloats, ra1, sl,
                                           (uint32_t*)(A + lay.bits[l]), stream));
        MOLCLR_TRY(molclr_gemm_f32_h3(a1, ra1, (int)molclr_gemm_row_parts(2 * D), p2, z, N, D,
                                      2 * D, 2 * D, D, MOLCLR_EPI_BIAS, e->mlp2_bias[l], nullptr, 0,
                                      nullptr,
                                      nullptr, nullptr, nullptr, stream));
      } else {
        if (h3)
          MOLCLR_TRY(molclr_gemm_f32_bplanes_max(agg, e->mlp0_planes[l], a1, N, 2 * D, D, D, 2 * D,
                                                 MOLCLR_EPI_BIAS_RELU, e->mlp0_bias[l], nullptr, 0,
                                                 fmax + 2 * l * kMaxSlotFloats,
                                                 fmax + (2 * l + 1) * kMaxSlotFloats, nullptr,
                                                 (uint32_t*)(A + lay.bits[l]), kws, kws_bytes,
// ... 434 lines not shown
```

molclr_amd/csrc/graph.hip:

```cpp
#include "common.h"
#include "stage.h"

namespace {

constexpr int kScanThreads = 1024;

struct GSegs {
  int n;
  const int64_t* ei[MOLCLR_MAX_SEGMENTS];
  const int64_t* ea[MOLCLR_MAX_SEGMENTS];
  const int64_t* batch[MOLCLR_MAX_SEGMENTS];
  int64_t n0[MOLCLR_MAX_SEGMENTS + 1], e0[MOLCLR_MAX_SEGMENTS + 1], g0[MOLCLR_MAX_SEGMENTS + 1];
  int64_t eld[MOLCLR_MAX_SEGMENTS];
  const int64_t* dcount;
};

__device__ __forceinline__ int gseg(const int64_t* off, int n, int64_t k) {
  int s = 0;
  while (s + 1 < n && k >= off[s + 1]) ++s;
  return s;
}

__device__ __forceinline__ int64_t gcount(const GSegs& sg, int which, int s) {
  if (sg.dcount) return sg.dcount[which * sg.n + s];
  return which ? sg.e0[s + 1] - sg.e0[s] : sg.n0[s + 1] - sg.n0[s];
}
__device__ __forceinline__ int64_t gbase(const GSegs& sg, int which, int s) {
  if (!sg.dcount) return which ? sg.e0[s] : sg.n0[s];
  int64_t b = 0;
  for (int q = 0; q < s; ++q) b += sg.dcount[which * sg.n + q];
  return b;
}
struct GLoc {
  int s;
  int64_t base, cnt;
};
__device__ __forceinline__ GLoc glocate(const GSegs& sg, int which, int64_t k) {
  int64_t b = 0;
  for (int s = 0; s < sg.n; ++s) {
    const int64_t c = gcount(sg, which, s);
    if (k < b + c) return {s, b, c};
    b += c;
  }
  return {-1, b, 0};
}

__global__ void k_graph_init(int32_t* __restrict__ ecount, int32_t* __restrict__ counters,
                             int64_t n_counters, int64_t N, int32_t* __restrict__ status) {
  int64_t t = (int64_t)blockIdx.x * blockDim.x + threadIdx.x;
  if (t == 0) *status = 0;
  if (t < n_counters) counters[t] = 0;
  if (t < N * MOLCLR_ECOUNT_STRIDE) {
    int j = (int)(t % MOLCLR_ECOUNT_STRIDE);
    ecount[t] = (j == MOLCLR_SELF_LOOP_BOND_TYPE || j == 5) ? 1 : 0;
  }
}

__device__ void graph_ptr_item(const GSegs& sg, int64_t t, int64_t N, int64_t G,
                               int32_t* __restrict__ graph_ptr, int32_t* __restrict__ status);

__global__ void k_graph_count(GSegs sg, int64_t E, int32_t* __restrict__ src32,
                              int32_t* __restrict__ dst32, uint8_t* __restrict__ code8,
                              int32_t* __restrict__ indeg, int32_t* __restrict__ outdeg,
                              int32_t* __restrict__ ecount, int32_t* __restrict__ status, int64_t N,
                              int64_t G, int32_t* __restrict__ graph_ptr) {
  int64_t k = (int64_t)blockIdx.x * blockDim.x + threadIdx.x;
  if (blockIdx.y == 1) {
    if (k < (N > G + 1 ? N : G + 1)) graph_ptr_item(sg, k, N, G, graph_ptr, status);
    return;
  }
  if (k >= E) return;
  const GLoc le = glocate(sg, 1, k);
  if (le.s < 0) return;
  const int g = le.s;
  const int64_t kk = k - le.base, Eg = le.cnt;
  const int64_t Ng = gcount(sg, 0, g), nb = gbase(sg, 0, g);
  const int64_t* ei = sg.ei[g];
  const int64_t* ea = sg.ea[g];
  int64_t s = ei[kk], d = ei[(sg.dcount ? sg.eld[g] : Eg) + kk];
  int64_t bt = ea[2 * kk], bd = ea[2 * kk + 1];
  int bad = 0;
  if (s < 0 || s >= Ng || d < 0 || d >= Ng) {
    bad |= 1;
    s = s < 0 ? 0 : (s >= Ng ? Ng - 1 : s);
    d = d < 0 ? 0 : (d >= Ng ? Ng - 1 : d);
  }
  if (bt < 0 || bt >= MOLCLR_NUM_BOND_TYPE || bd < 0 || bd >= MOLCLR_NUM_BOND_DIR) {
    bad |= 2;
    bt = bt < 0 ? 0 : (bt >= MOLCLR_NUM_BOND_TYPE ? MOLCLR_NUM_BOND_TYPE - 1 : bt);
    bd = bd < 0 ? 0 : (bd >= MOLCLR_NUM_BOND_DIR ? MOLCLR_NUM_BOND_DIR - 1 : bd);
  }
  if (bad) atomicOr(status, bad);
  s += nb;
  d += nb;
  src32[k] = (int32_t)s;
  dst32[k] = (int32_t)d;
  code8[k] = (uint8_t)(bt | (bd << 3));
  atomicAdd(&indeg[d], 1);
  atomicAdd(&outdeg[s], 1);
  atomicAdd(&ecount[d * MOLCLR_ECOUNT_STRIDE + bt], 1);
  atomicAdd(&ecount[d * MOLCLR_ECOUNT_STRIDE + 5 + bd], 1);
}

constexpr int kScanPer = 8;
__global__ __launch_bounds__(kScanThreads) void k_scan2(const int32_t* __restrict__ degA,
                                                        int32_t* __restrict__ ptrA,
                                                        const int32_t* __restrict__ degB,
                                                        int32_t* __restrict__ ptrB, int64_t n) {
  constexpr int TILE = kScanPer * kScanThreads;
  const int32_t* deg = blockIdx.y == 0 ? degA : degB;
  int32_t* ptr = blockIdx.y == 0 ? ptrA : ptrB;
  __shared__ int32_t tile[TILE];
  __shared__ int32_t wsum[kScanThreads / 64];
  const int tid = threadIdx.x, lane = tid & 63, wid = tid >> 6;
  const int64_t base = (int64_t)blockIdx.x * TILE;
  int32_t nx[kScanPer];
#pragma unroll
  for (int c = 0; c < kScanPer; ++c) {
    const int64_t idx = base + (int64_t)c * kScanThreads + tid;
    nx[c] = idx < n ? deg[idx] : 0;
  }
  int32_t pre = 0;
  for (int64_t i0 = tid; i0 < base; i0 += (int64_t)kScanPer * kScanThreads) {
    int32_t q[kScanPer];
#pragma unroll
    for (int c = 0; c < kScanPer; ++c) {
      const int64_t i = i0 + (int64_t)c * kScanThreads;
      q[c] = i < base ? deg[i] : 0;
    }
#pragma unroll
    for (int c = 0; c < kScanPer; ++c) pre += q[c];
  }
#pragma unroll
  for (int o = 32; o > 0; o >>= 1) pre += __shfl_xor(pre, o, 64);
  if (lane == 0) wsum[wid] = pre;
#pragma unroll
  for (int c = 0; c < kScanPer; ++c) tile[c * kScanThreads + tid] = nx[c];
  __syncthreads();
  int32_t carry = 0;
#pragma unroll
  for (int w = 0; w < kScanThreads / 64; ++w) carry += wsum[w];
  int32_t v[kScanPer], x = 0;
#pragma unroll
  for (int j = 0; j < kScanPer; ++j) {
    v[j] = tile[kScanPer * tid + j];
    x += v[j];
  }
  const int32_t own = x;
#pragma unroll
  for (int o = 1; o < 64; o <<= 1) {
    const int32_t u = __shfl_up(x, o, 64);
    if (lane >= o) x += u;
  }
  __syncthreads();
  if (lane == 63) wsum[wid] = x;
  __syncthreads();
  if (wid == 0) {
    int32_t w = lane < kScanThreads / 64 ? wsum[lane] : 0;
#pragma unroll
    for (int o = 1; o < 64; o <<= 1) {
      const int32_t u = __shfl_up(w, o, 64);
      if (lane >= o) w += u;
    }
    if (lane < kScanThreads / 64) wsum[lane] = w;
  }
  __syncthreads();
  int32_t run = carry + (wid > 0 ? wsum[wid - 1] : 0) + x - own;
#pragma unroll
  for (int j = 0; j < kScanPer; ++j) {
    const int64_t idx = base + (int64_t)kScanPer * tid + j;
    if (idx < n) ptr[idx] = run;
    run += v[j];
  }
  if (tid == 0 && base + TILE >= n) ptr[n] = carry + wsum[kScanThreads / 64 - 1];
}

__global__ void k_graph_fill(GSegs sg, const int32_t* __restrict__ src32,
                             const int32_t* __restrict__ dst32, int64_t E,
                             const int32_t* __restrict__ rowptr,
                             const int32_t* __restrict__ rowptr_t, int32_t* __restrict__ cur,
                             int32_t* __restrict__ cur_t, int32_t* __restrict__ perm,
                             int32_t* __restrict__ perm_t) {
  int64_t k = (int64_t)blockIdx.x * blockDim.x + threadIdx.x;
  if (k >= E || (sg.dcount && k >= gbase(sg, 1, sg.n))) return;
  int32_t s = src32[k], d = dst32[k];
  perm[rowptr[d] + atomicAdd(&cur[d], 1)] = (int32_t)k;
  perm_t[rowptr_t[s] + atomicAdd(&cur_t[s], 1)] = (int32_t)k;
}

__global__ void k_graph_rows(int64_t N, const int32_t* __restrict__ src32,
                             const int32_t* __restrict__ dst32, const uint8_t* __restrict__ code8,
                             const int32_t* __restrict__ rowptr, const int32_t* __restrict__ rowptr_t,
                             int32_t* __restrict__ perm, int32_t* __restrict__ perm_t,
                             int32_t* __restrict__ col, uint8_t* __restrict__ ecode,
                             int32_t* __restrict__ col_t, uint4* __restrict__ nbr,
                             uint4* __restrict__ nbr_t) {
  int64_t t = (int64_t)blockIdx.x * blockDim.x + threadIdx.x;
  if (t >= 2 * N) return;
  bool csc = t >= N;
  int64_t i = csc ? t - N : t;
  const int32_t* ptr = csc ? rowptr_t : rowptr;
  int32_t* p = csc ? perm_t : perm;
  int32_t beg = ptr[i], end = ptr[i + 1];
  for (int32_t a = beg + 1; a < end; ++a) {
    int32_t key = p[a];
    int32_t b = a - 1;
    while (b >= beg && p[b] > key) {
      p[b + 1] = p[b];
      --b;
    }
    p[b + 1] = key;
  }
  uint32_t slot[MOLCLR_NBR_SLOTS] = {0u, 0u, 0u, 0u};
  if (!csc) {
    for (int32_t a = beg; a < end; ++a) {
      int32_t k = p[a];
      col[a] = src32[k];
      ecode[a] = code8[k];
      if (a - beg < MOLCLR_NBR_SLOTS)
        slot[a - beg] = (uint32_t)src32[k] | ((uint32_t)MOLCLR_ECOMB(code8[k]) << 24);
    }
  } else {
    for (int32_t a = beg; a < end; ++a) {
      col_t[a] = dst32[p[a]];
      if (a - beg < MOLCLR_NBR_SLOTS) slot[a - beg] = (uint32_t)dst32[p[a]];
    }
  }
  const int32_t deg = end - beg;
  slot[0] |= (uint32_t)(deg > MOLCLR_NBR_SLOTS ? MOLCLR_NBR_OVERFLOW : deg) << 29;
  (csc ? nbr_t : nbr)[i] = make_uint4(slot[0], slot[1], slot[2], slot[3]);
}

__device__ void graph_ptr_item(const GSegs& sg, int64_t t, int64_t N, int64_t G,
                               int32_t* __restrict__ graph_ptr, int32_t* __restrict__ status) {
  if (t < N) {
    const GLoc ln = glocate(sg, 0, t);
    if (ln.s >= 0) {
      const int g = ln.s;
      const int64_t* batch = sg.batch[g];
      const int64_t i = t - ln.base, Gg = sg.g0[g + 1] - sg.g0[g];
      const int64_t b = batch[i];
      if (b < 0 || b >= Gg || (i > 0 && batch[i - 1] > b)) atomicOr(status, 4);
    }
  }
  if (t <= G) {
    if (t == G) {
      graph_ptr[t] = (int32_t)gbase(sg, 0, sg.n);
    } else {
      const int g = gseg(sg.g0, sg.n, t);
      const int64_t* batch = sg.batch[g];
      const int64_t want = t - sg.g0[g];
      int64_t lo = 0, hi = gcount(sg, 0, g);
      while (lo < hi) {
        int64_t mid = (lo + hi) >> 1;
        if (batch[mid] < want) lo = mid + 1;
        else hi = mid;
      }
      graph_ptr[t] = (int32_t)(gbase(sg, 0, g) + lo);
    }
  }
}

int build_launch(const GSegs& sg, int64_t N, int64_t E, int64_t G, int32_t* rowptr, int32_t* col,
                 uint8_t* ecode, int32_t* rowptr_t, int32_t* col_t, uint32_t* nbr, uint32_t* nbr_t,
                 int32_t* ecount, int32_t* graph_ptr, int32_t* status, void* workspace,
                 size_t workspace_bytes, molclr_stream_t stream) {
  MOLCLR_REQUIRE(rowptr && rowptr_t && ecount && graph_ptr && status && (N == 0 || (nbr && nbr_t)),
                 "graph_build: null output");
  MOLCLR_REQUIRE(E == 0 || (col && ecode && col_t), "graph_build: null edge buffer");
  MOLCLR_REQUIRE_WS(workspace_bytes, molclr_graph_build_workspace_bytes(N, E));
  hipStream_t s = molclr::as_stream(stream);
  molclr::Workspace w(workspace, workspace_bytes);
  int32_t* src32 = w.take<int32_t>(E);
  int32_t* dst32 = w.take<int32_t>(E);
  uint8_t* code8 = w.take<uint8_t>(E);
  int32_t* counters = w.take<int32_t>(4 * N);
  int32_t* indeg = counters;
  int32_t* outdeg = counters + N;
  int32_t* cur = counters + 2 * N;
  int32_t* cur_t = counters + 3 * N;
  int32_t* perm = w.take<int32_t>(E);
  int32_t* perm_t = w.take<int32_t>(E);

  const int T = 256;
  int64_t n_init = 8 * N > 4 * N ? 8 * N : 4 * N;
  if (n_init < 1) n_init = 1;
  hipLaunchKernelGGL(k_graph_init, dim3(molclr::ceil_div(n_init, T)), dim3(T), 0, s, ecount,
                     counters, 4 * N, N, status);
  const int64_t n_ptr = N > G + 1 ? N : G + 1;
  const int64_t bx = molclr::ceil_div(E > n_ptr ? E : n_ptr, T);
  hipLaunchKernelGGL(k_graph_count, dim3((unsigned)bx, 2), dim3(T), 0, s, sg, E, src32, dst32,
                     code8, indeg, outdeg, ecount, status, N, G, graph_ptr);
  hipLaunchKernelGGL(k_scan2,
                     dim3((unsigned)(N > 0 ? molclr::ceil_div(N, kScanPer * kScanThreads) : 1), 2),
                     dim3(kScanThreads), 0, s, indeg, rowptr, outdeg, rowptr_t, N);
  if (E > 0) {
    hipLaunchKernelGGL(k_graph_fill, dim3(molclr::ceil_div(E, T)), dim3(T), 0, s, sg, src32, dst32,
                       E, rowptr, rowptr_t, cur, cur_t, perm, perm_t);
  }
  if (N > 0) {
    hipLaunchKernelGGL(k_graph_rows, dim3(molclr::ceil_div(2 * N, T)), dim3(T), 0, s, N, src32,
                       dst32, code8, rowptr, rowptr_t, perm, perm_t, col, ecode, col_t,
                       (uint4*)nbr, (uint4*)nbr_t);
  }
  MOLCLR_LAUNCHED();
  return MOLCLR_OK;
}

}

MOLCLR_API size_t molclr_graph_build_workspace_bytes(int64_t N, int64_t E) {
  molclr::Workspace w(nullptr, 0);
  w.take<int32_t>(E);
  w.take<int32_t>(E);
  w.take<uint8_t>(E);
  w.take<int32_t>(4 * N);
  w.take<int32_t>(E);
  w.take<int32_t>(E);
  return w.used + 256;
}

MOLCLR_API int molclr_graph_build_multi(int nseg, const molclr_graph_segment* segs,
                                        int32_t* rowptr, int32_t* col, uint8_t* ecode,
                                        int32_t* rowptr_t, int32_t* col_t, uint32_t* nbr,
                                        uint32_t* nbr_t, int32_t* ecount, int32_t* graph_ptr,
                                        int32_t* status, void* workspace, size_t workspace_bytes,
                                        molclr_stream_t stream) {
  MOLCLR_REQUIRE(nseg >= 1 && nseg <= MOLCLR_MAX_SEGMENTS && segs,
                 "graph_build: %d segments (1..%d)", nseg, MOLCLR_MAX_SEGMENTS);
  GSegs sg{};
  sg.n = nseg;
  for (int g = 0; g < nseg; ++g) {
    const molclr_graph_segment& q = segs[g];
    MOLCLR_REQUIRE(q.num_nodes >= 0 && q.num_edges >= 0 && q.num_graphs >= 0,
                   "graph_build: negative size in segment %d", g);
    sg.ei[g] = q.edge_index;
    sg.ea[g] = q.edge_attr;
    sg.batch[g] = q.batch;
    sg.n0[g + 1] = sg.n0[g] + q.num_nodes;
    sg.e0[g + 1] = sg.e0[g] + q.num_edges;
    sg.g0[g + 1] = sg.g0[g] + q.num_graphs;
  }
  for (int g = nseg; g < MOLCLR_MAX_SEGMENTS; ++g) {
    sg.n0[g + 1] = sg.n0[nseg];
    sg.e0[g + 1] = sg.e0[nseg];
    sg.g0[g + 1] = sg.g0[nseg];
  }
  const int64_t N = sg.n0[nseg], E = sg.e0[nseg], G = sg.g0[nseg];
  MOLCLR_REQUIRE(N <= MOLCLR_NBR_MAX_NODES && E < (int64_t)1 << 31,
                 "graph_build: %lld nodes exceed the neighbour-slot limit %d (or E > int32)",
                 (long long)N, MOLCLR_NBR_MAX_NODES);
  for (int g = 0; g < nseg; ++g) {
    MOLCLR_REQUIRE(segs[g].num_edges == 0 || (segs[g].edge_index && segs[g].edge_attr),
                   "graph_build: null edge input in segment %d", g);
    MOLCLR_REQUIRE(segs[g].num_nodes == 0 || segs[g].batch, "graph_build: null batch in segment %d",
                   g);
  }
  return build_launch(sg, N, E, G, rowptr, col, ecode, rowptr_t, col_t, nbr, nbr_t, ecount,
                      graph_ptr, status, workspace, workspace_bytes, stream);
}

MOLCLR_API int molclr_graph_build(const int64_t* edge_index, const int64_t* edge_attr,
                                  const int64_t* batch, int64_t N, int64_t E, int64_t G,
                                  int32_t* rowptr, int32_t* col, uint8_t* ecode,
                                  int32_t* rowptr_t, int32_t* col_t, uint32_t* nbr,
                                  uint32_t* nbr_t, int32_t* ecount, int32_t* graph_ptr,
                                  int32_t* status, void* workspace,
                                  size_t workspace_bytes, molclr_stream_t stream) {
  const molclr_graph_segment seg{edge_index, edge_attr, batch, N, E, G};
  return molclr_graph_build_multi(1, &seg, rowptr, col, ecode, rowptr_t, col_t, nbr, nbr_t, ecount,
                                  graph_ptr, status, workspace, workspace_bytes, stream);
}

MOLCLR_API int molclr_stage_segments(int nseg, const molclr_stage_source* src,
                                     const molclr_graph_staged_segment* dst, int64_t* x_all,
                                     int64_t num_nodes_cap, int64_t num_edges_cap,
                                     int64_t* counts, molclr_stream_t stream) {
  molclr::StageJobs jb{};
  int nj = 0;
  int64_t most = 1;
  MOLCLR_TRY_RC(molclr::stage_plan("stage_segments", nseg, src, dst, x_all, num_nodes_cap,
                                   num_edges_cap, counts, jb, nj, most));
  molclr::stage_launch(jb, nj, most, molclr::as_stream(stream));
  MOLCLR_LAUNCHED();
  return MOLCLR_OK;
}

MOLCLR_API int molclr_graph_build_dev(int nseg, const molclr_graph_staged_segment* segs,
                                      const int64_t* counts, int64_t num_nodes_cap,
                                      int64_t num_edges_cap, int32_t* rowptr, int32_t* col,
                                      uint8_t* ecode, int32_t* rowptr_t, int32_t* col_t,
                                      uint32_t* nbr, uint32_t* nbr_t, int32_t* ecount,
                                      int32_t* graph_ptr, int32_t* status, void* workspace,
                                      size_t workspace_bytes, molclr_stream_t stream) {
  MOLCLR_REQUIRE(nseg >= 1 && nseg <= MOLCLR_MAX_SEGMENTS && segs && counts,
                 "graph_build_dev: %d segments (1..%d)", nseg, MOLCLR_MAX_SEGMENTS);
  GSegs sg{};
  sg.n = nseg;
  sg.dcount = counts;
  int64_t ecap = 0;
  for (int g = 0; g < nseg; ++g) {
    const molclr_graph_staged_segment& q = segs[g];
    MOLCLR_REQUIRE(q.node_cap >= 0 && q.edge_cap >= 0 && q.num_graphs >= 0 &&
                       q.edge_index && q.edge_attr && q.batch,
                   "graph_build_dev: bad segment %d", g);
    sg.ei[g] = q.edge_index;
    sg.ea[g] = q.edge_attr;
    sg.batch[g] = q.batch;
    sg.eld[g] = q.edge_cap;
    sg.g0[g + 1] = sg.g0[g] + q.num_graphs;
    ecap += q.edge_cap;
  }
  for (int g = nseg; g < MOLCLR_MAX_SEGMENTS; ++g) sg.g0[g + 1] = sg.g0[nseg];
  const int64_t N = num_nodes_cap, E = num_edges_cap, G = sg.g0[nseg];
  MOLCLR_REQUIRE(E >= 1 && E <= ecap,
                 "graph_build_dev: num_edges_cap %lld must be in [1, sum of edge_cap %lld]",
                 (long long)E, (long long)ecap);
  MOLCLR_REQUIRE(N >= 1 && N <= MOLCLR_NBR_MAX_NODES && E < (int64_t)1 << 31,
                 "graph_build_dev: %lld nodes exceed the neighbour-slot limit %d (or E > int32)",
                 (long long)N, MOLCLR_NBR_MAX_NODES);
  return build_launch(sg, N, E, G, rowptr, col, ecode, rowptr_t, col_t, nbr, nbr_t, ecount,
                      graph_ptr, status, workspace, workspace_bytes, stream);
}
```

molclr_amd/csrc/norm.hip:

```cpp
#include "common.h"

#include <math.h>

namespace {

constexpr int kT = 256;

__host__ __device__ __forceinline__ int64_t band_parts(int64_t rows, int band) {
  const int64_t unit = (int64_t)band * 16;
  int64_t P = (rows + unit - 1) / unit;
  if (P > 1024) P = 1024;
  if (P < 1) P = 1;
  return P;
}

int64_t band_parts_bound(int64_t rows, int band, int nseg) {
  const int64_t unit = (int64_t)band * 16;
  int64_t P = (rows + unit - 1) / unit + nseg;
  if (P > (int64_t)nseg * 1024) P = (int64_t)nseg * 1024;
  return P;
}

template <typename St = StF32>
__global__ void k_colsum_partial(const typename St::T* __restrict__ X, int64_t rows, int d4,
// ... 731 lines not shown
  }
  for (int32_t i = beg; i < end; ++i) St::st(dh, (int64_t)i * d4 + c, v);
}

template <typename St = StF32>
__global__ void k_pool_max_fwd(const typename St::T* __restrict__ h, const int32_t* __restrict__ ptr,
                               float4* __restrict__ out, int4* __restrict__ arg, int64_t G, int d4) {
  int64_t t = (int64_t)blockIdx.x * blockDim.x + threadIdx.x;
  if (t >= G * d4) return;
  int64_t g = t / d4;
  int c = (int)(t - g * d4);
  int32_t beg = ptr[g], end = ptr[g + 1];
  float m[4] = {-INFINITY, -INFINITY, -INFINITY, -INFINITY};
  int a[4] = {-1, -1, -1, -1};
  for (int32_t i = beg; i < end; ++i) {
    const float4 v = St::ld(h, (int64_t)i * d4 + c);
    const float e[4] = {v.x, v.y, v.z, v.w};
#pragma unroll
    for (int j = 0; j < 4; ++j)
      if (a[j] < 0 || e[j] > m[j]) {
        m[j] = e[j];
        a[j] = i;
      }
  }
#pragma unroll
  for (int j = 0; j < 4; ++j)
    if (a[j] < 0) m[j] = 0.f;
  out[t] = make_float4(m[0], m[1], m[2], m[3]);
  arg[t] = make_int4(a[0], a[1], a[2], a[3]);
}

template <typename St = StF32>
__global__ void k_pool_max_bwd(const float4* __restrict__ dout, const int4* __restrict__ arg,
                               typename St::T* __restrict__ dh, int64_t G, int d4) {
  int64_t t = (int64_t)blockIdx.x * blockDim.x + threadIdx.x;
  if (t >= G * d4) return;
  const int c = (int)(t % d4);
  const float4 v = dout[t];
  const int4 a = arg[t];
  const float e[4] = {v.x, v.y, v.z, v.w};
  const int ai[4] = {a.x, a.y, a.z, a.w};
#pragma unroll
  for (int j = 0; j < 4; ++j)
    if (ai[j] >= 0) St::st1(dh, (int64_t)ai[j] * (4 * d4) + 4 * c + j, e[j]);
}

__global__ __launch_bounds__(256) void k_l2norm_fwd(const float* __restrict__ z,
                                                    float* __restrict__ y,
                                                    float* __restrict__ norm, int64_t rows,
                                                    int64_t D, float eps) {
  const int lane = threadIdx.x & 63;
  const int64_t r = ((int64_t)blockIdx.x * blockDim.x + threadIdx.x) >> 6;
  if (r >= rows) return;
  const float* zr = z + r * D;
  float ss = 0.f;
  for (int64_t c = lane; c < D; c += 64) ss += zr[c] * zr[c];
  ss = wave_sum(ss);
  float nrm = sqrtf(ss);
  float den = fmaxf(nrm, eps);
  if (lane == 0) norm[r] = nrm;
  for (int64_t c = lane; c < D; c += 64) y[r * D + c] = zr[c] / den;
}

__global__ __launch_bounds__(256) void k_l2norm_bwd(const float* __restrict__ dy,
                                                    const float* __restrict__ y,
                                                    const float* __restrict__ norm,
                                                    float* __restrict__ dz, int64_t rows,
                                                    int64_t D, float eps) {
  const int lane = threadIdx.x & 63;
  const int64_t r = ((int64_t)blockIdx.x * blockDim.x + threadIdx.x) >> 6;
  if (r >= rows) return;
  float nrm = norm[r];
  if (nrm > eps) {
    float dot = 0.f;
    for (int64_t c = lane; c < D; c += 64) dot += dy[r * D + c] * y[r * D + c];
    dot = wave_sum(dot);
    for (int64_t c = lane; c < D; c += 64)
      dz[r * D + c] = (dy[r * D + c] - dot * y[r * D + c]) / nrm;
  } else {
    for (int64_t c = lane; c < D; c += 64) dz[r * D + c] = dy[r * D + c] / eps;
  }
}

__global__ __launch_bounds__(1024) void k_sum(const float* __restrict__ x, float* __restrict__ out,
                                              int64_t n) {
  __shared__ float ws[16];
  float acc = 0.f;
  for (int64_t i = threadIdx.x; i < n; i += blockDim.x) acc += x[i];
  acc = wave_sum(acc);
  if ((threadIdx.x & 63) == 0) ws[threadIdx.x >> 6] = acc;
  __syncthreads();
  if (threadIdx.x == 0) {
    float s = 0.f;
    for (int w = 0; w < (int)(blockDim.x >> 6); ++w) s += ws[w];
    *out = s;
  }
}

}

size_t molclr_colsum_ws(int64_t rows, int64_t cols) {
  if (!molclr::band_dim_ok(cols)) return 0;
  molclr::Band b = molclr::make_band(cols);
  return (size_t)band_parts(rows, b.band) * cols * sizeof(float) + 256;
}

int molclr_colsum_impl(const void* X, int dtype, float* out, int64_t rows, int64_t cols,
                       int64_t ld, int accumulate, molclr::Workspace& w, hipStream_t s) {
  MOLCLR_REQUIRE(molclr::band_dim_ok(cols),
                 "colsum: cols %lld must be a multiple of 4 in [4, %lld]", (long long)cols,
                 (long long)molclr::kBandMaxDim);
  MOLCLR_REQUIRE(ld % 4 == 0, "colsum: ld %lld must be a multiple of 4", (long long)ld);
  molclr::Band b = molclr::make_band(cols);
  int64_t P = band_parts(rows, b.band);
  float* partial = w.take<float>(P * cols);
  if (!w.ok()) {
    molclr::set_error("colsum: workspace too small");
    return MOLCLR_ERR_WORKSPACE;
  }
  int64_t rpp = molclr::ceil_div(rows > 0 ? rows : 1, P);
  size_t lds = (size_t)b.band * b.d4 * sizeof(float4);
  if (dtype == MOLCLR_DTYPE_BF16)
    hipLaunchKernelGGL(k_colsum_partial<StBF16>, dim3(P), dim3(b.threads), lds, s,
                       (const uint16_t*)X, rows, b.d4, ld / 4, b.band, rpp, (float4*)partial);
  else
    hipLaunchKernelGGL(k_colsum_partial<StF32>, dim3(P), dim3(b.threads), lds, s, (const float*)X,
                       rows, b.d4, ld / 4, b.band, rpp, (float4*)partial);
  hipLaunchKernelGGL(k_colsum_final, dim3(molclr::ceil_div(cols, kRedCols)), dim3(kRedCols * kRedLanes), 0, s, partial, P,
                     cols, out, accumulate);
  MOLCLR_LAUNCHED();
  return MOLCLR_OK;
}

MOLCLR_API size_t molclr_colsum_f32_workspace_bytes(int64_t rows, int64_t cols) {
  return molclr_colsum_ws(rows, cols);
}

MOLCLR_API int molclr_colsum_f32(const float* X, float* out, int64_t rows, int64_t cols,
                                 int64_t ld, int accumulate, void* workspace,
                                 size_t workspace_bytes, molclr_stream_t stream) {
  MOLCLR_REQUIRE(molclr::band_dim_ok(cols),
                 "colsum: cols %lld must be a multiple of 4 in [4, %lld]", (long long)cols,
                 (long long)molclr::kBandMaxDim);
  MOLCLR_REQUIRE_WS(workspace_bytes, molclr_colsum_ws(rows, cols));
  molclr::Workspace w(workspace, workspace_bytes);
  return molclr_colsum_impl(X, MOLCLR_DTYPE_F32, out, rows, cols, ld, accumulate, w,
                            molclr::as_stream(stream));
}

namespace {

using molclr::BnBwdArgs;
using molclr::BnFwdArgs;
using molclr::BnSegs;

struct BnPlan {
  Segs sg;
  molclr::Band b;
  int64_t P, rows;
};
int make_plan(int nseg, const int64_t* seg_rows, const int64_t* drows, int64_t cap, int64_t D,
              BnPlan& p) {
  MOLCLR_REQUIRE(nseg >= 1 && nseg <= MOLCLR_MAX_SEGMENTS && (seg_rows || drows),
                 "batchnorm: %d segments (1..%d)", nseg, MOLCLR_MAX_SEGMENTS);
  MOLCLR_REQUIRE(molclr::band_dim_ok(D), "batchnorm: dim %lld must be a multiple of 4 in [4, %lld]",
                 (long long)D, (long long)molclr::kBandMaxDim);
  p.b = molclr::make_band(D);
  Segs& sg = p.sg;
  sg.n = nseg;
  sg.band = p.b.band;
  sg.drows = drows;
  p.P = 0;
  p.rows = 0;
  for (int s = 0; s < MOLCLR_MAX_SEGMENTS; ++s) sg.rows[s] = 0;
  if (drows) {
    MOLCLR_REQUIRE(cap >= 0, "batchnorm: negative row capacity");
    p.P = band_parts_bound(cap, p.b.band, nseg);
    p.rows = cap;
    return MOLCLR_OK;
// ... 442 lines not shown
  if (N == 0) return MOLCLR_OK;
  const int d4 = (int)(D / 4);
  const int64_t work = G * d4 > 0 ? G * d4 : 1;
  hipLaunchKernelGGL(k_pool_bwd<StBF16>, dim3(molclr::ceil_div(work, kT)), dim3(kT), 0, s,
                     (const float4*)dout, graph_ptr, dh, G, d4, mode, N);
  MOLCLR_LAUNCHED();
  return MOLCLR_OK;
}

MOLCLR_API int molclr_segment_max_fwd(const void* h, const int32_t* graph_ptr, float* out,
                                      int32_t* argmax, int64_t G, int64_t D, int dtype,
                                      molclr_stream_t stream) {
  MOLCLR_REQUIRE(D > 0 && D % 4 == 0, "segment_max_fwd: dim must be a multiple of 4");
  MOLCLR_REQUIRE(dtype == MOLCLR_DTYPE_F32 || dtype == MOLCLR_DTYPE_BF16,
                 "segment_max_fwd: bad dtype %d", dtype);
  MOLCLR_REQUIRE(G >= 0, "segment_max_fwd: bad graph count");
  if (G == 0) return MOLCLR_OK;
  MOLCLR_REQUIRE(h && graph_ptr && out && argmax, "segment_max_fwd: null pointer");
  const int d4 = (int)(D / 4);
  const dim3 g(molclr::ceil_div(G * d4, kT)), b(kT);
  hipStream_t s = molclr::as_stream(stream);
  if (dtype == MOLCLR_DTYPE_BF16)
    hipLaunchKernelGGL(k_pool_max_fwd<StBF16>, g, b, 0, s, static_cast<const uint16_t*>(h),
                       graph_ptr, (float4*)out, (int4*)argmax, G, d4);
  else
    hipLaunchKernelGGL(k_pool_max_fwd<StF32>, g, b, 0, s, static_cast<const float*>(h), graph_ptr,
                       (float4*)out, (int4*)argmax, G, d4);
  MOLCLR_LAUNCHED();
  return MOLCLR_OK;
}

MOLCLR_API int molclr_segment_max_bwd(const float* dout, const int32_t* argmax, void* dh,
                                      int64_t N, int64_t G, int64_t D, int dtype,
                                      molclr_stream_t stream) {
  MOLCLR_REQUIRE(D > 0 && D % 4 == 0, "segment_max_bwd: dim must be a multiple of 4");
  MOLCLR_REQUIRE(dtype == MOLCLR_DTYPE_F32 || dtype == MOLCLR_DTYPE_BF16,
                 "segment_max_bwd: bad dtype %d", dtype);
  MOLCLR_REQUIRE(N >= 0 && G >= 0, "segment_max_bwd: bad sizes");
  hipStream_t s = molclr::as_stream(stream);
  const size_t esz = dtype == MOLCLR_DTYPE_BF16 ? sizeof(uint16_t) : sizeof(float);
  if (N > 0 && molclr::zero_async(dh, (size_t)N * D * esz, s) != hipSuccess) {
    molclr::set_error("segment_max_bwd: memset failed");
    return MOLCLR_ERR_ARG;
  }
  if (G == 0) return MOLCLR_OK;
  const int d4 = (int)(D / 4);
  const dim3 g(molclr::ceil_div(G * d4, kT)), b(kT);
  if (dtype == MOLCLR_DTYPE_BF16)
    hipLaunchKernelGGL(k_pool_max_bwd<StBF16>, g, b, 0, s, (const float4*)dout,
                       (const int4*)argmax, static_cast<uint16_t*>(dh), G, d4);
  else
    hipLaunchKernelGGL(k_pool_max_bwd<StF32>, g, b, 0, s, (const float4*)dout, (const int4*)argmax,
                       static_cast<float*>(dh), G, d4);
  MOLCLR_LAUNCHED();
  return MOLCLR_OK;
}

MOLCLR_API int molclr_l2norm_fwd(const float* z, float* y, float* norm, int64_t rows, int64_t D,
                                 double eps, molclr_stream_t stream) {
  MOLCLR_REQUIRE(D > 0, "l2norm_fwd: bad dim");
  if (rows == 0) return MOLCLR_OK;
  hipLaunchKernelGGL(k_l2norm_fwd, dim3(molclr::ceil_div(rows * 64, 256)), dim3(256), 0,
                     molclr::as_stream(stream), z, y, norm, rows, D, (float)eps);
  MOLCLR_LAUNCHED();
  return MOLCLR_OK;
}

MOLCLR_API int molclr_l2norm_bwd(const float* dy, const float* y, const float* norm, float* dz,
                                 int64_t rows, int64_t D, double eps, molclr_stream_t stream) {
  MOLCLR_REQUIRE(D > 0, "l2norm_bwd: bad dim");
  if (rows == 0) return MOLCLR_OK;
  hipLaunchKernelGGL(k_l2norm_bwd, dim3(molclr::ceil_div(rows * 64, 256)), dim3(256), 0,
                     molclr::as_stream(stream), dy, y, norm, dz, rows, D, (float)eps);
  MOLCLR_LAUNCHED();
  return MOLCLR_OK;
}

MOLCLR_API int molclr_sum_f32(const float* x, float* out, int64_t n, molclr_stream_t stream) {
  MOLCLR_REQUIRE(out && (n == 0 || x), "sum_f32: null pointer");
  hipLaunchKernelGGL(k_sum, dim3(1), dim3(1024), 0, molclr::as_stream(stream), x, out, n);
  MOLCLR_LAUNCHED();
  return MOLCLR_OK;
}
```

molclr_amd/graph_step.py:

```python
from __future__ import annotations

import ctypes
from collections import OrderedDict

import torch

from . import _lib, ops
from .data import DeviceGraph, _num_graphs_of


def _round_up(n: int, q: int) -> int:
    return max(q, (int(n) + q - 1) // q * q)


class StagedPairGraph(DeviceGraph):

    def __init__(self, device, node_cap: int, edge_cap: int, graphs_per_segment):
        self.device = device
        self.nseg = len(graphs_per_segment)
        i64 = dict(dtype=torch.long, device=device)
        i32 = dict(dtype=torch.int32, device=device)
        N, E, G = int(node_cap), int(edge_cap), int(sum(graphs_per_segment))
        self.num_nodes, self.num_edges, self.num_graphs = N, E, G
        self.graphs_per_segment = [int(g) for g in graphs_per_segment]
        self.segment_nodes = None
        self.st_ei = [torch.zeros(2, E, **i64) for _ in range(self.nseg)]
        self.st_ea = [torch.zeros(E, 2, **i64) for _ in range(self.nseg)]
        self.st_batch = [torch.zeros(N, **i64) for _ in range(self.nseg)]
        self.x = torch.zeros(N, 2, **i64)
        self.counts = torch.zeros(2 * self.nseg, **i64)
        self._dst = (_lib.StagedSegmentC * self.nseg)()
        for q in range(self.nseg):
            self._dst[q] = _lib.StagedSegmentC(self.st_ei[q].data_ptr(), self.st_ea[q].data_ptr(),
                                               self.st_batch[q].data_ptr(), N, E,
                                               self.graphs_per_segment[q])
        self.rowptr = torch.empty(N + 1, **i32)
        self.col = torch.empty(E, **i32)
        self.ecode = torch.empty(E, dtype=torch.uint8, device=device)
        self.rowptr_t = torch.empty(N + 1, **i32)
        self.col_t = torch.empty(E, **i32)
        self.nbr = torch.empty(N * 4, **i32)
        self.nbr_t = torch.empty(N * 4, **i32)
        self.ecount = torch.empty(N * 8, **i32)
        self.graph_ptr = torch.empty(G + 1, **i32)
        self.status = torch.zeros(1, **i32)
        self._ws_bytes = _lib.query("molclr_graph_build_workspace_bytes", N, E)
        self._ws = torch.empty(self._ws_bytes, dtype=torch.uint8, device=device)
        self._keep = []

    def fits(self, views) -> bool:
        n = sum(int(v.x.shape[0]) for v in views)
        e = sum(int(v.edge_index.shape[1]) for v in views)
        return (n <= self.num_nodes and e <= self.num_edges
                and [_num_graphs_of(v) for v in views] == self.graphs_per_segment)

    def stage(self, views) -> None:
        if len(views) != self.nseg:
            raise ValueError(f"StagedPairGraph: {len(views)} views, built for {self.nseg}")
        src = (_lib.StageSourceC * self.nseg)()
        keep = []
        for q, d in enumerate(views):
            if _num_graphs_of(d) != self.graphs_per_segment[q]:
                raise ValueError("StagedPairGraph: a view's graph count changed "
                                 f"({_num_graphs_of(d)} vs {self.graphs_per_segment[q]})")
            x = d.x.to(torch.long).contiguous()
            ei = d.edge_index.to(torch.long).contiguous()
            ea = d.edge_attr.to(torch.long).contiguous()
            b = getattr(d, "batch", None)
            if b is None:
                b = torch.zeros(x.shape[0], dtype=torch.long, device=x.device)
            b = b.to(torch.long).contiguous()
            keep += [x, ei, ea, b]
            src[q] = _lib.StageSourceC(x.data_ptr(), ei.data_ptr(), ea.data_ptr(), b.data_ptr(),
                                       int(x.shape[0]), int(ei.shape[1]))
        _lib.call("molclr_stage_segments", self.nseg, ctypes.addressof(src),
                  ctypes.addressof(self._dst), self.x.data_ptr(), self.num_nodes, self.num_edges,
                  self.counts.data_ptr(), _lib.stream_of(self.device))
        self._keep = keep

    def build(self) -> None:
        _lib.call("molclr_graph_build_dev", self.nseg, ctypes.addressof(self._dst),
                  self.counts.data_ptr(), self.num_nodes, self.num_edges,
                  self.rowptr.data_ptr(), self.col.data_ptr(), self.ecode.data_ptr(),
                  self.rowptr_t.data_ptr(), self.col_t.data_ptr(), self.nbr.data_ptr(),
                  self.nbr_t.data_ptr(), self.ecount.data_ptr(), self.graph_ptr.data_ptr(),
                  self.status.data_ptr(), self._ws.data_ptr(), self._ws_bytes,
                  _lib.stream_of(self.device))

    def cstruct(self):
        c = getattr(self, "_cstruct", None)
        if c is None:
            c = _lib.DeviceGraphC(self.num_nodes, self.num_edges, self.num_graphs, *[
                t.data_ptr() for t in (self.rowptr, self.col, self.rowptr_t, self.col_t,
                                       self.ecount, self.graph_ptr, self.ecode, self.nbr,
                                       self.nbr_t)])
            c.num_segments = self.nseg
            c.segment_nodes_dev = self.counts.data_ptr()
            self._cstruct = c
        return c


class _Captured:
    def __init__(self, graph: StagedPairGraph, cuda_graph, keep=()):
        self.graph = graph
        self.cuda_graph = cuda_graph
        self.keep = list(keep)


def _drain_collectives(*groups) -> None:
    import torch.distributed as dist
    if not (dist.is_available() and dist.is_initialized()):
        return
    seen = set()
    for g in (*groups, dist.group.WORLD):
        if g is None or id(g) in seen:
            continue
        seen.add(id(g))
        wait = getattr(g, "_wait_for_pending_works", None)
        if wait is not None:
            wait()


class CapturedTrainStep:

    def __init__(self, model, optimizer, criterion, node_quantum: int = 256,
                 edge_quantum: int = 2048, max_graphs: int = 16, node_slack: int | None = None,
                 edge_headroom: float = 0.04, reducer=None):
        from .optim import FusedAdam
        if not isinstance(optimizer, FusedAdam):
            raise TypeError("CapturedTrainStep needs molclr_amd.optim.FusedAdam "
                            "(learning rate and step counter on the device)")
        if not hasattr(model, "forward_staged"):
            raise TypeError("CapturedTrainStep: the model has no forward_staged")
        self.group = getattr(criterion, "group", None)
        if reducer is not None and reducer.flat is not optimizer.flat_grad:
            raise ValueError("CapturedTrainStep: the reducer must reduce this optimizer's gradients")
        self.reducer = reducer
        self.model, self.optimizer, self.criterion = model, optimizer, criterion
        self.node_quantum, self.edge_quantum = int(node_quantum), int(edge_quantum)
        self.node_slack = 2 * self.node_quantum if node_slack is None else int(node_slack)
        self.edge_headroom = float(edge_headroom)
        self.max_graphs = int(max_graphs)
        self.device = optimizer.flat.device
        self._graphs: OrderedDict = OrderedDict()
        self.loss = torch.zeros((), dtype=torch.float32, device=self.device)
        self.status = torch.zeros(1, dtype=torch.int32, device=self.device)
        self.captures = 0
        self.replays = 0
        self.eager_steps = 0
        self._one = None
        self.last_graph: StagedPairGraph | None = None

    @staticmethod
    def _need(xis, xjs) -> tuple:
        n = int(xis.x.shape[0]) + int(xjs.x.shape[0])
        e = int(xis.edge_index.shape[1]) + int(xjs.edge_index.shape[1])
        return n, e, _num_graphs_of(xis), _num_graphs_of(xjs)

    def bucket(self, xis, xjs) -> tuple:
        n, e, gi, gj = self._need(xis, xjs)
        e_cap = _round_up(int(e * (1.0 + self.edge_headroom)) + 1, self.edge_quantum)
        return (_round_up(n, self.node_quantum), e_cap, gi, gj)

    def lookup(self, xis, xjs):
        n, e, gi, gj = self._need(xis, xjs)
        limit = _round_up(n, self.node_quantum) + self.node_slack
        best = None
        for ent in self._graphs.values():
            g = ent.graph
            if (g.num_nodes >= n and g.num_edges >= e and g.num_nodes <= limit
                    and g.graphs_per_segment == [gi, gj]):
                if best is None or (g.num_nodes, g.num_edges) < (best.graph.num_nodes,
                                                                 best.graph.num_edges):
                    best = ent
        return best

    def _capture(self, key, pair=None) -> _Captured:
        if not self.model._executor_ok() or self.model._dim_pad():
            raise NotImplementedError(
                "CapturedTrainStep: the model must run through the encoder executor with "
                "emb_dim a multiple of the kernels' width (tracked BatchNorm)")
        ops._check_no_timer()
        graph = StagedPairGraph(self.device, key[0], key[1], key[2:])
        if pair is not None:
            graph.stage(list(pair))
        opt = self.optimizer
        opt.sync_lr()
        ops.bump_param_generation()
        g = torch.cuda.CUDAGraph()
        torch.cuda.synchronize(self.device)
        _drain_collectives(self.group, getattr(self.reducer, "group", None))
        mode = "global" if self.group is None else "thread_local"
        self._dry_run(graph)
        ops.CAPTURE_SCOPE = {id(p) for p in self.model.parameters()}
        ops.CAPTURE_KEEP = keep = []
        try:
            self._record(g, mode, graph, opt)
        finally:
            ops.CAPTURE_SCOPE = None
            ops.CAPTURE_KEEP = None
        if self.reducer is not None:
            keep += self.reducer.capture_events
        self.captures += 1
        ops.bump_param_generation()
        return _Captured(graph, g, keep)

    def _dry_run(self, graph):
        from . import _lib
        if self._one is None:
            self._one = torch.ones((), dtype=torch.float32, device=self.device)
        with _lib.dry_run():
            _, z = self.model.forward_staged(graph)
            loss = self.criterion.forward_pair_normalized(z)
            loss.backward(self._one)
        del loss, z
        ops.bump_param_generation()
        torch.cuda.synchronize(self.device)

    def _record(self, g, mode, graph, opt):
        with torch.cuda.graph(g, pool=torch.cuda.graph_pool_handle(), capture_error_mode=mode):
            graph.build()
            opt.zero_grad()
            if self.reducer is not None:
                self.reducer.arm()
            _, z = self.model.forward_staged(graph)
            loss = self.criterion.forward_pair_normalized(z)
            loss.backward(self._one)
            if self.reducer is not None:
                self.reducer.finish()
            elif self.group is not None:
                from .distributed import allreduce_grads
                allreduce_grads(opt.flat_grad, self.group)
            opt.step(sync_lr=False, tick=False)
            _lib.call("molclr_step_tail", opt._step_dev.data_ptr(), loss.data_ptr(),
                      self.loss.data_ptr(), graph.status.data_ptr(), self.status.data_ptr(),
                      _lib.stream_of(self.device))
        del loss, z

    def _insert(self, ent) -> None:
        self._graphs[id(ent)] = ent
        if len(self._graphs) > self.max_graphs:
            self._graphs.popitem(last=False)

    def _entry(self, xis, xjs):
        ent = self.lookup(xis, xjs)
        if ent is None:
            ent = self._capture(self.bucket(xis, xjs), (xis, xjs))
            self._insert(ent)
            return ent, True
        if not self._multi_rank():
            self._graphs.move_to_end(id(ent))
        return ent, False

    def _multi_rank(self) -> bool:
        import torch.distributed as dist
        return (self.group is not None and dist.is_available() and dist.is_initialized()
                and dist.get_world_size(self.group) > 1)

    def _global_sizes(self, sizes) -> list:
        import torch.distributed as dist
        loc = torch.tensor([[int(a), int(b)] for a, b in sizes] or [[0, 0]],
                           dtype=torch.long, device=self.device)[: max(len(sizes), 1)]
        n = torch.tensor([len(sizes)], dtype=torch.long, device=self.device)
        ns = [torch.zeros_like(n) for _ in range(dist.get_world_size(self.group))]
        dist.all_gather(ns, n, group=self.group)
        most = max(1, max(int(t.item()) for t in ns))
        pad = torch.zeros(most, 2, dtype=torch.long, device=self.device)
        pad[: loc.shape[0]] = loc
        outs = [torch.zeros_like(pad) for _ in ns]
        dist.all_gather(outs, pad, group=self.group)
        return sorted({(int(a), int(b)) for o, k in zip(outs, ns)
                       for a, b in o[: int(k.item())].tolist()}, reverse=True)

    def prepare(self, pairs) -> int:
        before = self.captures
        pairs = list(pairs)
        if self._multi_rank():
            sizes = [self._need(a, b)[:2] for a, b in pairs]
            gi = {self._need(a, b)[2] for a, b in pairs}
            gj = {self._need(a, b)[3] for a, b in pairs}
            if len(gi) != 1 or len(gj) != 1:
                raise ValueError("CapturedTrainStep.prepare: data parallel batches must hold a "
                                 "fixed number of molecules per view")
            return self.prepare_sizes(sizes, gi.pop(), gj.pop())
        for xis, xjs in pairs:
            self._entry(xis, xjs)
        return self.captures - before

    def prepare_sizes(self, sizes, graphs_i: int, graphs_j: int) -> int:
        before = self.captures
        if self._multi_rank():
            sizes = self._global_sizes(list(sizes))

        class _V:
            def __init__(self, n, e, g):
                self.x = torch.empty(n, 0)
                self.edge_index = torch.empty(2, e)
                self._num_graphs = g

            @property
            def num_graphs(self):
                return self._num_graphs

        for n, e in sorted(((int(a), int(b)) for a, b in sizes), reverse=True):
            vi, vj = _V(n, e, graphs_i), _V(0, 0, graphs_j)
            if self.lookup(vi, vj) is None:
                self._insert(self._capture(self.bucket(vi, vj)))
        return self.captures - before

    def _eager(self, xis, xjs) -> torch.Tensor:
        from .data import pair_graph
        opt = self.optimizer
        opt.zero_grad()
        if self.reducer is not None:
            self.reducer.arm()
        _, z = self.model.forward_pair(xis, xjs)
        loss = self.criterion.forward_pair_normalized(z)
        loss.backward()
        if self.reducer is not None:
# ... 100 lines not shown
```

molclr_amd/ops.py:

```python
from __future__ import annotations

import torch

import contextlib
import ctypes
import dataclasses
import os
import functools
import weakref

from . import _lib
from ._lib import EPI_ACCUMULATE, EPI_BIAS, EPI_BIAS_RELU, EPI_NONE, EPI_RELU_MASK
from .data import DeviceGraph


@functools.lru_cache(maxsize=4096)
def _wsq(name: str, *args) -> int:
    return _lib.query(name, *args)


def _grad_sink(param, shape, device):
    if param is not None and getattr(param, "_molclr_fused_grad", False) and param.grad is not None:
        return param.grad, 1, None
    t = torch.empty(shape, dtype=torch.float32, device=device)
# ... 739 lines not shown


class _L2Normalize(torch.autograd.Function):
    @staticmethod
    def forward(ctx, z, eps):
        _check(z)
        z = _c(z)
        rows, D = z.shape
        y = torch.empty_like(z)
        norm = torch.empty(rows, dtype=torch.float32, device=z.device)
        _lib.call("molclr_l2norm_fwd", z.data_ptr(), y.data_ptr(), norm.data_ptr(), rows, D,
                  float(eps), _stream(z))
        ctx.save_for_backward(y, norm)
        ctx.eps = eps
        return y

    @staticmethod
    def backward(ctx, dy):
        y, norm = ctx.saved_tensors
        dy = _c(dy)
        rows, D = y.shape
        dz = torch.empty_like(y)
        _lib.call("molclr_l2norm_bwd", dy.data_ptr(), y.data_ptr(), norm.data_ptr(), dz.data_ptr(),
                  rows, D, float(ctx.eps), _stream(dy))
        return dz, None


_GIDX: dict = {}


def _row_index(n, dev, group):
    if group is None:
        key, rank, world = (n, dev.index, 0, 1), 0, 1
    else:
        import torch.distributed as dist
        rank, world = dist.get_rank(group), dist.get_world_size(group)
        key = (n, dev.index, rank, world)
    g = _GIDX.get(key)
    if g is not None:
        return g
    if group is None:
        g = torch.arange(n, dtype=torch.int32, device=dev)
    else:
        from . import distributed as mdist
        g = mdist.global_row_index(n // 2, rank, world, dev)
    if not torch.cuda.is_current_stream_capturing():
        _GIDX[key] = g
    return g


def _ntxent_rows_forward(ctx, rhat, batch_size, temperature, group):
    dev = rhat.device
    n, C = rhat.shape
    Bl = n // 2
    st = _lib.stream_of(dev)
    if group is None:
        B = Bl
        if batch_size != B:
            raise ValueError(f"NTXentLoss built for batch_size={batch_size} got {B} rows "
                             "(the reference requires full batches, dataset.py:179)")
        cols = rhat
    else:
        import torch.distributed as dist

        from . import distributed as mdist
        B = Bl * dist.get_world_size(group)
        if batch_size != B:
            raise ValueError(f"global batch {B} != NTXentLoss batch_size {batch_size}")
        cols = mdist.gather_rows(rhat, group)
    gidx = _row_index(n, dev, group)
    lse = torch.empty(n, dtype=torch.float32, device=dev)
    loss_rows = torch.empty(n, dtype=torch.float32, device=dev)
    ws_bytes = _wsq("molclr_ntxent_workspace_bytes", n, 2 * B, C)
    ws = _ws(ws_bytes, dev)
    sim_bytes = _wsq("molclr_ntxent_sim_bytes", n, 2 * B, C, -1)
    sim = (torch.empty(sim_bytes // 4, dtype=torch.float32, device=dev) if sim_bytes
           else torch.empty(0, dtype=torch.float32, device=dev))
    _lib.call("molclr_ntxent_fwd_impl", rhat.data_ptr(), gidx.data_ptr(), cols.data_ptr(), n,
              2 * B, C, B, float(temperature), lse.data_ptr(), loss_rows.data_ptr(),
              sim.data_ptr() if sim_bytes else None, ws.data_ptr(), ws_bytes, st, -1)
    if _TIMER is not None:
        _TIMER.add("ntxent", 2.0 * n * 2 * B * C)
    loss = torch.empty((), dtype=torch.float32, device=dev)
    _lib.call("molclr_sum_f32", loss_rows.data_ptr(), loss.data_ptr(), n, st)
    if group is None:
        lse_cols = lse
    else:
        from . import distributed as mdist
        lse_cols, loss = mdist.gather_lse_and_sum(lse, loss, group)
    ctx.ntx = (B, C, float(temperature))
    return loss, (cols, gidx, lse_cols, sim)


def _ntxent_rows_backward(ctx, rhat, gloss, cols, gidx, lse_cols, sim):
    B, C, T = ctx.ntx
    dev = rhat.device
    n = rhat.shape[0]
    gloss = gloss.to(torch.float32).contiguous()
    drhat = torch.empty_like(rhat)
    ws_bytes = _wsq("molclr_ntxent_workspace_bytes", n, 2 * B, C)
    ws = _ws(ws_bytes, dev)
    _lib.call("molclr_ntxent_bwd_impl", rhat.data_ptr(), gidx.data_ptr(), cols.data_ptr(),
              lse_cols.data_ptr(), gloss.data_ptr(), n, 2 * B, C, B, T,
              sim.data_ptr() if sim.numel() else None, drhat.data_ptr(), ws.data_ptr(),
              ws_bytes, _lib.stream_of(dev), -1)
    if _TIMER is not None:
        _TIMER.add("ntxent", (2.0 if sim.numel() else 4.0) * n * 2 * B * C)
    return drhat


class _NTXent(torch.autograd.Function):

    @staticmethod
    def forward(ctx, R, batch_size, temperature, cosine, group):
        _check(R)
        R = _c(R)
        n, C = R.shape
        rhat = torch.empty_like(R)
        norm = torch.empty(n, dtype=torch.float32, device=R.device)
        _lib.call("molclr_ntxent_prep", R.data_ptr(), rhat.data_ptr(), norm.data_ptr(), n, C,
                  int(cosine), _lib.stream_of(R.device))
        loss, kept = _ntxent_rows_forward(ctx, rhat, batch_size, temperature, group)
        ctx.save_for_backward(rhat, norm, *kept)
        ctx.cosine = int(cosine)
        return loss

    @staticmethod
    def backward(ctx, gloss):
        rhat, norm, *kept = ctx.saved_tensors
        n, C = rhat.shape
        drhat = _ntxent_rows_backward(ctx, rhat, gloss, *kept)
        dR = torch.empty_like(rhat)
        _lib.call("molclr_ntxent_prep_bwd", drhat.data_ptr(), rhat.data_ptr(), norm.data_ptr(),
                  dR.data_ptr(), n, C, ctx.cosine, _lib.stream_of(rhat.device))
        return dR, None, None, None, None


class _NTXentPairNormalized(torch.autograd.Function):

    @staticmethod
    def forward(ctx, z, batch_size, temperature, cosine, group, eps):
        _check(z)
        z = _c(z)
        n, C = z.shape
        dev = z.device
        y = torch.empty_like(z)
        rhat = torch.empty_like(z)
        n1 = torch.empty(n, dtype=torch.float32, device=dev)
        n2 = torch.empty(n, dtype=torch.float32, device=dev)
        _lib.call("molclr_ntxent_prep_pair", z.data_ptr(), y.data_ptr(), rhat.data_ptr(),
                  n1.data_ptr(), n2.data_ptr(), n // 2, C, float(eps), int(cosine),
                  _lib.stream_of(dev))
        loss, kept = _ntxent_rows_forward(ctx, rhat, batch_size, temperature, group)
        ctx.save_for_backward(y, rhat, n1, n2, *kept)
        ctx.cosine, ctx.eps = int(cosine), float(eps)
        return loss

    @staticmethod
    def backward(ctx, gloss):
        y, rhat, n1, n2, *kept = ctx.saved_tensors
        n, C = rhat.shape
        drhat = _ntxent_rows_backward(ctx, rhat, gloss, *kept)
        dz = torch.empty_like(rhat)
        _lib.call("molclr_ntxent_prep_pair_bwd", drhat.data_ptr(), rhat.data_ptr(), n2.data_ptr(),
                  y.data_ptr(), n1.data_ptr(), dz.data_ptr(), n // 2, C, ctx.eps, ctx.cosine,
                  _lib.stream_of(rhat.device))
        return dz, None, None, None, None, None


DTYPES = {"fp32": _lib.DTYPE_F32, "bf16": _lib.DTYPE_BF16}
TORCH_DTYPE = {_lib.DTYPE_F32: torch.float32, _lib.DTYPE_BF16: torch.bfloat16}


@dataclasses.dataclass(frozen=True)
# ... 627 lines not shown
```

Baseline: 196,000 molecules/s.

## Fold small launches: fuse embed with edge tables, loss sum with step tail, graph init

```diff
diff --git a/include/molclr.h b/include/molclr.h
--- a/include/molclr.h
+++ b/include/molclr.h
@@ -77,6 +77,13 @@
                            uint32_t* nbr, uint32_t* nbr_t, int32_t* ecount, int32_t* graph_ptr,
                            int32_t* status, void* workspace, size_t workspace_bytes,
                            molclr_stream_t stream);
+int molclr_graph_build_dev_resident(int nseg, const molclr_graph_staged_segment* segs,
+                                    const int64_t* counts, int64_t num_nodes_cap,
+                                    int64_t num_edges_cap, int32_t* rowptr, int32_t* col,
+                                    uint8_t* ecode, int32_t* rowptr_t, int32_t* col_t,
+                                    uint32_t* nbr, uint32_t* nbr_t, int32_t* ecount,
+                                    int32_t* graph_ptr, int32_t* status, void* workspace,
+                                    size_t workspace_bytes, molclr_stream_t stream);
 
 size_t molclr_mask_views_workspace_bytes(int64_t batch_size);
 int molclr_mask_views(const int64_t* store_x, const int64_t* store_atom_ptr,
@@ -127,6 +134,11 @@
 #define MOLCLR_MAX_LAYERS 16
 int molclr_edge_tables_combine(int layers, const float* const* E1s, const float* const* E2s,
                                float* Ec, int64_t dim, molclr_stream_t stream);
+int molclr_atom_embed_fwd_tables(const int64_t* x, const float* X1, const float* X2, float* h,
+                                 int64_t num_nodes, int64_t dim, int64_t n1, int64_t n2,
+                                 int32_t* status, int layers, const float* const* E1s,
+                                 const float* const* E2s, float* Ec, float* zero, int64_t n_zero,
+                                 molclr_stream_t stream);
 
 int molclr_gine_aggregate_fwd(const float* x, const int32_t* rowptr, const int32_t* col,
                               const uint8_t* ecode, const uint32_t* nbr, const float* Ec,
@@ -427,6 +439,8 @@
                         double eps, double weight_decay, int tick, molclr_stream_t stream);
 int molclr_step_tail(int32_t* step, const float* loss_src, float* loss_dst,
                      const int32_t* status_src, int32_t* status_acc, molclr_stream_t stream);
+int molclr_sum_step_tail(const float* x, int64_t n, float* loss, float* loss_dst, int32_t* step,
+                         const int32_t* status_src, int32_t* status_acc, molclr_stream_t stream);
 
 enum {
   MOLCLR_MODE_EVAL = 0,
diff --git a/molclr_amd/_lib.py b/molclr_amd/_lib.py
--- a/molclr_amd/_lib.py
+++ b/molclr_amd/_lib.py
@@ -23,6 +23,8 @@
     "molclr_stage_segments": (c_int, [c_int, _P, _P, _P, _I64, _I64, _P, _P]),
     "molclr_graph_build_dev": (c_int, [c_int, _P, _P, _I64, _I64, _P, _P, _P, _P, _P, _P, _P, _P,
                                        _P, _P, _P, c_size_t, _P]),
+    "molclr_graph_build_dev_resident": (c_int, [c_int, _P, _P, _I64, _I64, _P, _P, _P, _P, _P, _P,
+                                                _P, _P, _P, _P, _P, c_size_t, _P]),
     "molclr_mask_views_workspace_bytes": (c_size_t, [_I64]),
     "molclr_mask_views": (c_int, [_P, _P, _P, _P, _P, _I64, _I64, _P, _I64, c_uint64, c_int, _P, _P,
                                   _P, _P, _P, _I64, _I64, _P, _P, c_size_t, _P]),
@@ -31,6 +33,8 @@
     "molclr_atom_embed_bwd": (c_int, [_P, _P, _P, _P, _I64, _I64, _I64, _I64, c_int, _P, c_size_t,
                                       _P]),
     "molclr_edge_tables_combine": (c_int, [c_int, _P, _P, _P, _I64, _P]),
+    "molclr_atom_embed_fwd_tables": (c_int, [_P, _P, _P, _P, _I64, _I64, _I64, _I64, _P, c_int, _P,
+                                             _P, _P, _P, _I64, _P]),
     "molclr_gine_aggregate_fwd": (c_int, [_P, _P, _P, _P, _P, _P, _P, _I64, _I64, _P]),
     "molclr_rowmax_layout": (_I64, [_I64]),
     "molclr_rowmax_bytes": (c_size_t, [_I64, _I64]),
@@ -150,6 +154,7 @@
     "molclr_adam_step_ex": (c_int, [_P, _P, _P, _P, _I64, _P, _P, c_double, c_double, c_double,
                                     c_double, c_int, _P]),
     "molclr_step_tail": (c_int, [_P, _P, _P, _P, _P, _P]),
+    "molclr_sum_step_tail": (c_int, [_P, _I64, _P, _P, _P, _P, _P, _P]),
     "molclr_gin_encoder_arena_bytes": (c_size_t, [c_int, _I64, _I64, c_int]),
     "molclr_gin_encoder_workspace_bytes": (c_size_t, [c_int, _I64, _I64, c_int]),
     "molclr_gin_encoder_fwd": (c_int, [_P, _P, _P, _P, _P, c_size_t, _P, c_size_t, _P]),
diff --git a/molclr_amd/csrc/aggregate.hip b/molclr_amd/csrc/aggregate.hip
--- a/molclr_amd/csrc/aggregate.hip
+++ b/molclr_amd/csrc/aggregate.hip
@@ -7,11 +7,12 @@
 constexpr int kT = 256;
 
 template <typename St, int U = 1>
-__global__ void k_atom_embed_fwd(const int64_t* __restrict__ x, const float4* __restrict__ X1,
-                                 const float4* __restrict__ X2, typename St::T* __restrict__ h,
-                                 int64_t N, int d4, int64_t n1, int64_t n2,
-                                 int32_t* __restrict__ status) {
-  int64_t t = (int64_t)blockIdx.x * blockDim.x + threadIdx.x;
+__device__ __forceinline__ void atom_embed_item(int64_t t, const int64_t* __restrict__ x,
+                                                const float4* __restrict__ X1,
+                                                const float4* __restrict__ X2,
+                                                typename St::T* __restrict__ h, int64_t N, int d4,
+                                                int64_t n1, int64_t n2,
+                                                int32_t* __restrict__ status) {
   if (t >= N * d4 / U) return;
   const int64_t u0 = t * U;
   int64_t i = N * d4 < (1ll << 32) ? (int64_t)((uint32_t)u0 / (uint32_t)d4) : u0 / d4;
@@ -29,6 +30,14 @@
   }
   if constexpr (U == 2) St::st2(h, t, v[0], v[1]);
   else St::st(h, t, v[0]);
+}
+template <typename St, int U = 1>
+__global__ void k_atom_embed_fwd(const int64_t* __restrict__ x, const float4* __restrict__ X1,
+                                 const float4* __restrict__ X2, typename St::T* __restrict__ h,
+                                 int64_t N, int d4, int64_t n1, int64_t n2,
+                                 int32_t* __restrict__ status) {
+  atom_embed_item<St, U>((int64_t)blockIdx.x * blockDim.x + threadIdx.x, x, X1, X2, h, N, d4, n1,
+                         n2, status);
 }
 
 constexpr int kEmbBlock = 256;
@@ -244,10 +253,10 @@
   const float* e1[MOLCLR_MAX_LAYERS];
   const float* e2[MOLCLR_MAX_LAYERS];
 };
-__global__ void k_edge_tables_combine(TablePtrs p, float* __restrict__ Ec, int layers, int64_t D,
-                                      float* __restrict__ zero, int64_t n_zero) {
+__device__ __forceinline__ void edge_tables_item(int64_t t, const TablePtrs& p,
+                                                 float* __restrict__ Ec, int layers, int64_t D,
+                                                 float* __restrict__ zero, int64_t n_zero) {
   const int64_t per = (int64_t)MOLCLR_NUM_ECOMB * D;
-  int64_t t = (int64_t)blockIdx.x * blockDim.x + threadIdx.x;
   if (t < n_zero) zero[t] = 0.f;
   if (t >= layers * per) return;
   const int l = (int)(t / per);
@@ -255,6 +264,22 @@
   const int r = (int)(rc / D);
   const int64_t c = rc - (int64_t)r * D;
   Ec[t] = p.e1[l][(r / 3) * D + c] + p.e2[l][(r % 3) * D + c];
+}
+__global__ void k_edge_tables_combine(TablePtrs p, float* __restrict__ Ec, int layers, int64_t D,
+                                      float* __restrict__ zero, int64_t n_zero) {
+  edge_tables_item((int64_t)blockIdx.x * blockDim.x + threadIdx.x, p, Ec, layers, D, zero, n_zero);
+}
+__global__ void k_atom_embed_tables(const int64_t* __restrict__ x, const float4* __restrict__ X1,
+                                    const float4* __restrict__ X2, float* __restrict__ h, int64_t N,
+                                    int d4, int64_t n1, int64_t n2, int32_t* __restrict__ status,
+                                    int64_t eb, TablePtrs p, float* __restrict__ Ec, int layers,
+                                    float* __restrict__ zero, int64_t n_zero) {
+  if ((int64_t)blockIdx.x < eb)
+    atom_embed_item<StF32, 1>((int64_t)blockIdx.x * blockDim.x + threadIdx.x, x, X1, X2, h, N, d4,
+                              n1, n2, status);
+  else
+    edge_tables_item(((int64_t)blockIdx.x - eb) * blockDim.x + threadIdx.x, p, Ec, layers,
+                     (int64_t)4 * d4, zero, n_zero);
 }
 
 __device__ __forceinline__ uint32_t nbr_degree(uint32_t w0) { return w0 >> 29; }
@@ -979,6 +1004,37 @@
   const int64_t work = n > n_zero ? n : n_zero;
   hipLaunchKernelGGL(k_edge_tables_combine, dim3(molclr::ceil_div(work, kT)), dim3(kT), 0,
                      molclr::as_stream(stream), p, Ec, layers, D, zero, n_zero);
+  MOLCLR_LAUNCHED();
+  return MOLCLR_OK;
+}
+
+MOLCLR_API int molclr_atom_embed_fwd_tables(const int64_t* x, const float* X1, const float* X2,
+                                            float* h, int64_t N, int64_t D, int64_t n1, int64_t n2,
+                                            int32_t* status, int layers, const float* const* E1s,
+                                            const float* const* E2s, float* Ec, float* zero,
+                                            int64_t n_zero, molclr_stream_t stream) {
+  MOLCLR_REQUIRE(D > 0 && D % 4 == 0, "atom_embed_fwd_tables: dim %lld must be a positive multiple of 4",
+                 (long long)D);
+  MOLCLR_REQUIRE(n1 > 0 && n2 > 0, "atom_embed_fwd_tables: empty table");
+  MOLCLR_REQUIRE(layers >= 1 && layers <= MOLCLR_MAX_LAYERS && E1s && E2s && Ec,
+                 "atom_embed_fwd_tables: %d layers (1..%d) or null tables", layers,
+                 MOLCLR_MAX_LAYERS);
+  MOLCLR_REQUIRE(N >= 0 && (N == 0 || (x && X1 && X2 && h)), "atom_embed_fwd_tables: null pointer");
+  MOLCLR_REQUIRE(n_zero >= 0 && (n_zero == 0 || zero), "atom_embed_fwd_tables: null zero range");
+  TablePtrs p{};
+  for (int l = 0; l < layers; ++l) {
+    MOLCLR_REQUIRE(E1s[l] && E2s[l], "atom_embed_fwd_tables: null table of layer %d", l);
+    p.e1[l] = E1s[l];
+    p.e2[l] = E2s[l];
+  }
+  const int d4 = (int)(D / 4);
+  const int64_t eb = molclr::ceil_div(N * d4, kT);
+  const int64_t n = (int64_t)layers * MOLCLR_NUM_ECOMB * D;
+  const int64_t tb = molclr::ceil_div(n > n_zero ? n : n_zero, kT);
+  MOLCLR_REQUIRE(eb + tb < (1ll << 31), "atom_embed_fwd_tables: too many rows");
+  hipLaunchKernelGGL(k_atom_embed_tables, dim3((unsigned)(eb + tb)), dim3(kT), 0,
+                     molclr::as_stream(stream), x, (const float4*)X1, (const float4*)X2, h, N, d4,
+                     n1, n2, status, eb, p, Ec, layers, zero, n_zero);
   MOLCLR_LAUNCHED();
   return MOLCLR_OK;
 }
diff --git a/molclr_amd/csrc/encoder.hip b/molclr_amd/csrc/encoder.hip
--- a/molclr_amd/csrc/encoder.hip
+++ b/molclr_amd/csrc/encoder.hip
@@ -6,6 +6,10 @@
 
 bool agg_bn() {
   static const bool on = !molclr::env_is("MOLCLR_AGG_BN", '0');
+  return on;
+}
+bool embed_tables() {
+  static const bool on = !molclr::env_is("MOLCLR_EMBED_TABLES", '0');
   return on;
 }
 
@@ -254,13 +258,19 @@
   if (bf)
     MOLCLR_TRY(molclr_atom_embed_fwd_bf16(x, e->x_embedding1, e->x_embedding2, (uint16_t*)h, N, D,
                                           e->n_atom, e->n_chiral, e->status, stream));
-  else
+  else if (!embed_tables())
     MOLCLR_TRY(molclr_atom_embed_fwd(x, e->x_embedding1, e->x_embedding2, (float*)h, N, D,
                                      e->n_atom, e->n_chiral, e->status, stream));
   float* Ec = F(lay.ec);
   const int64_t nz = h3 ? (int64_t)(lay.bmax - lay.smax) / 4 + (int64_t)L * 2 * kMaxSlotFloats : 0;
-  MOLCLR_TRY(molclr::edge_tables_combine_zero(L, e->edge_embedding1, e->edge_embedding2, Ec, D,
-                                              h3 ? fmax : nullptr, nz, stream));
+  if (!bf && embed_tables())
+    MOLCLR_TRY(molclr_atom_embed_fwd_tables(x, e->x_embedding1, e->x_embedding2, (float*)h, N, D,
+                                            e->n_atom, e->n_chiral, e->status, L,
+                                            e->edge_embedding1, e->edge_embedding2, Ec,
+                                            h3 ? fmax : nullptr, nz, stream));
+  else
+    MOLCLR_TRY(molclr::edge_tables_combine_zero(L, e->edge_embedding1, e->edge_embedding2, Ec, D,
+                                                h3 ? fmax : nullptr, nz, stream));
   for (int l = 0; l < L; ++l) {
     const bool last = l == L - 1;
     const bool bn_src = fused && l > 0;
diff --git a/molclr_amd/csrc/graph.hip b/molclr_amd/csrc/graph.hip
--- a/molclr_amd/csrc/graph.hip
+++ b/molclr_amd/csrc/graph.hip
@@ -98,6 +98,7 @@
   code8[k] = (uint8_t)(bt | (bd << 3));
   atomicAdd(&indeg[d], 1);
   atomicAdd(&outdeg[s], 1);
+  if (ecount == nullptr) return;
   atomicAdd(&ecount[d * MOLCLR_ECOUNT_STRIDE + bt], 1);
   atomicAdd(&ecount[d * MOLCLR_ECOUNT_STRIDE + 5 + bd], 1);
 }
@@ -106,8 +107,14 @@
 __global__ __launch_bounds__(kScanThreads) void k_scan2(const int32_t* __restrict__ degA,
                                                         int32_t* __restrict__ ptrA,
                                                         const int32_t* __restrict__ degB,
-                                                        int32_t* __restrict__ ptrB, int64_t n) {
+                                                        int32_t* __restrict__ ptrB, int64_t n,
+                                                        int32_t* __restrict__ flag,
+                                                        int32_t* __restrict__ status) {
   constexpr int TILE = kScanPer * kScanThreads;
+  if (flag != nullptr && blockIdx.x == 0 && blockIdx.y == 0 && threadIdx.x == 0) {
+    *status = *flag;
+    *flag = 0;
+  }
   const int32_t* deg = blockIdx.y == 0 ? degA : degB;
   int32_t* ptr = blockIdx.y == 0 ? ptrA : ptrB;
   __shared__ int32_t tile[TILE];
@@ -194,7 +201,8 @@
                              int32_t* __restrict__ perm, int32_t* __restrict__ perm_t,
                              int32_t* __restrict__ col, uint8_t* __restrict__ ecode,
                              int32_t* __restrict__ col_t, uint4* __restrict__ nbr,
-                             uint4* __restrict__ nbr_t) {
+                             uint4* __restrict__ nbr_t, int32_t* __restrict__ ecount,
+                             int32_t* __restrict__ counters) {
   int64_t t = (int64_t)blockIdx.x * blockDim.x + threadIdx.x;
   if (t >= 2 * N) return;
   bool csc = t >= N;
@@ -212,11 +220,15 @@
     p[b + 1] = key;
   }
   uint32_t slot[MOLCLR_NBR_SLOTS] = {0u, 0u, 0u, 0u};
+  int32_t ec[MOLCLR_ECOUNT_STRIDE] = {0, 0, 0, 0, 1, 1, 0, 0};
   if (!csc) {
     for (int32_t a = beg; a < end; ++a) {
       int32_t k = p[a];
       col[a] = src32[k];
       ecode[a] = code8[k];
+      const int bt = code8[k] & 7, bd = 5 + (code8[k] >> 3);
+#pragma unroll
+      for (int j = 0; j < MOLCLR_ECOUNT_STRIDE; ++j) ec[j] += (j == bt) + (j == bd);
       if (a - beg < MOLCLR_NBR_SLOTS)
         slot[a - beg] = (uint32_t)src32[k] | ((uint32_t)MOLCLR_ECOMB(code8[k]) << 24);
     }
@@ -229,6 +241,13 @@
   const int32_t deg = end - beg;
   slot[0] |= (uint32_t)(deg > MOLCLR_NBR_SLOTS ? MOLCLR_NBR_OVERFLOW : deg) << 29;
   (csc ? nbr_t : nbr)[i] = make_uint4(slot[0], slot[1], slot[2], slot[3]);
+  if (ecount == nullptr) return;
+  if (!csc) {
+#pragma unroll
+    for (int j = 0; j < MOLCLR_ECOUNT_STRIDE; ++j) ecount[i * MOLCLR_ECOUNT_STRIDE + j] = ec[j];
+  }
+  counters[(csc ? N : 0) + i] = 0;
+  counters[(csc ? 3 * N : 2 * N) + i] = 0;
 }
 
 __device__ void graph_ptr_item(const GSegs& sg, int64_t t, int64_t N, int64_t G,
@@ -264,7 +283,7 @@
 int build_launch(const GSegs& sg, int64_t N, int64_t E, int64_t G, int32_t* rowptr, int32_t* col,
                  uint8_t* ecode, int32_t* rowptr_t, int32_t* col_t, uint32_t* nbr, uint32_t* nbr_t,
                  int32_t* ecount, int32_t* graph_ptr, int32_t* status, void* workspace,
-                 size_t workspace_bytes, molclr_stream_t stream) {
+                 size_t workspace_bytes, molclr_stream_t stream, bool resident = false) {
   MOLCLR_REQUIRE(rowptr && rowptr_t && ecount && graph_ptr && status && (N == 0 || (nbr && nbr_t)),
                  "graph_build: null output");
   MOLCLR_REQUIRE(E == 0 || (col && ecode && col_t), "graph_build: null edge buffer");
@@ -281,19 +300,25 @@
   int32_t* cur_t = counters + 3 * N;
   int32_t* perm = w.take<int32_t>(E);
   int32_t* perm_t = w.take<int32_t>(E);
+  int32_t* flag = w.take<int32_t>(1);
+  int32_t* no_i32 = nullptr;
 
   const int T = 256;
-  int64_t n_init = 8 * N > 4 * N ? 8 * N : 4 * N;
-  if (n_init < 1) n_init = 1;
-  hipLaunchKernelGGL(k_graph_init, dim3(molclr::ceil_div(n_init, T)), dim3(T), 0, s, ecount,
-                     counters, 4 * N, N, status);
+  if (!resident) {
+    int64_t n_init = 8 * N > 4 * N ? 8 * N : 4 * N;
+    if (n_init < 1) n_init = 1;
+    hipLaunchKernelGGL(k_graph_init, dim3(molclr::ceil_div(n_init, T)), dim3(T), 0, s, ecount,
+                       counters, 4 * N, N, status);
+  }
   const int64_t n_ptr = N > G + 1 ? N : G + 1;
   const int64_t bx = molclr::ceil_div(E > n_ptr ? E : n_ptr, T);
   hipLaunchKernelGGL(k_graph_count, dim3((unsigned)bx, 2), dim3(T), 0, s, sg, E, src32, dst32,
-                     code8, indeg, outdeg, ecount, status, N, G, graph_ptr);
+                     code8, indeg, outdeg, resident ? no_i32 : ecount, resident ? flag : status, N,
+                     G, graph_ptr);
   hipLaunchKernelGGL(k_scan2,
                      dim3((unsigned)(N > 0 ? molclr::ceil_div(N, kScanPer * kScanThreads) : 1), 2),
-                     dim3(kScanThreads), 0, s, indeg, rowptr, outdeg, rowptr_t, N);
+                     dim3(kScanThreads), 0, s, indeg, rowptr, outdeg, rowptr_t, N,
+                     resident ? flag : no_i32, status);
   if (E > 0) {
     hipLaunchKernelGGL(k_graph_fill, dim3(molclr::ceil_div(E, T)), dim3(T), 0, s, sg, src32, dst32,
                        E, rowptr, rowptr_t, cur, cur_t, perm, perm_t);
@@ -301,7 +326,7 @@
   if (N > 0) {
     hipLaunchKernelGGL(k_graph_rows, dim3(molclr::ceil_div(2 * N, T)), dim3(T), 0, s, N, src32,
                        dst32, code8, rowptr, rowptr_t, perm, perm_t, col, ecode, col_t,
-                       (uint4*)nbr, (uint4*)nbr_t);
+                       (uint4*)nbr, (uint4*)nbr_t, resident ? ecount : no_i32, counters);
   }
   MOLCLR_LAUNCHED();
   return MOLCLR_OK;
@@ -317,6 +342,7 @@
   w.take<int32_t>(4 * N);
   w.take<int32_t>(E);
   w.take<int32_t>(E);
+  w.take<int32_t>(1);
   return w.used + 256;
 }
 
@@ -386,13 +412,12 @@
   return MOLCLR_OK;
 }
 
-MOLCLR_API int molclr_graph_build_dev(int nseg, const molclr_graph_staged_segment* segs,
-                                      const int64_t* counts, int64_t num_nodes_cap,
-                                      int64_t num_edges_cap, int32_t* rowptr, int32_t* col,
-                                      uint8_t* ecode, int32_t* rowptr_t, int32_t* col_t,
-                                      uint32_t* nbr, uint32_t* nbr_t, int32_t* ecount,
-                                      int32_t* graph_ptr, int32_t* status, void* workspace,
-                                      size_t workspace_bytes, molclr_stream_t stream) {
+namespace {
+int build_dev(int nseg, const molclr_graph_staged_segment* segs, const int64_t* counts,
+              int64_t num_nodes_cap, int64_t num_edges_cap, int32_t* rowptr, int32_t* col,
+              uint8_t* ecode, int32_t* rowptr_t, int32_t* col_t, uint32_t* nbr, uint32_t* nbr_t,
+              int32_t* ecount, int32_t* graph_ptr, int32_t* status, void* workspace,
+              size_t workspace_bytes, molclr_stream_t stream, bool resident) {
   MOLCLR_REQUIRE(nseg >= 1 && nseg <= MOLCLR_MAX_SEGMENTS && segs && counts,
                  "graph_build_dev: %d segments (1..%d)", nseg, MOLCLR_MAX_SEGMENTS);
   GSegs sg{};
@@ -420,5 +445,31 @@
                  "graph_build_dev: %lld nodes exceed the neighbour-slot limit %d (or E > int32)",
                  (long long)N, MOLCLR_NBR_MAX_NODES);
   return build_launch(sg, N, E, G, rowptr, col, ecode, rowptr_t, col_t, nbr, nbr_t, ecount,
-                      graph_ptr, status, workspace, workspace_bytes, stream);
-}
+                      graph_ptr, status, workspace, workspace_bytes, stream, resident);
+}
+}
+
+MOLCLR_API int molclr_graph_build_dev(int nseg, const molclr_graph_staged_segment* segs,
+                                      const int64_t* counts, int64_t num_nodes_cap,
+                                      int64_t num_edges_cap, int32_t* rowptr, int32_t* col,
+                                      uint8_t* ecode, int32_t* rowptr_t, int32_t* col_t,
+                                      uint32_t* nbr, uint32_t* nbr_t, int32_t* ecount,
+                                      int32_t* graph_ptr, int32_t* status, void* workspace,
+                                      size_t workspace_bytes, molclr_stream_t stream) {
+  return build_dev(nseg, segs, counts, num_nodes_cap, num_edges_cap, rowptr, col, ecode, rowptr_t,
+                   col_t, nbr, nbr_t, ecount, graph_ptr, status, workspace, workspace_bytes, stream,
+                   false);
+}
+
+MOLCLR_API int molclr_graph_build_dev_resident(int nseg, const molclr_graph_staged_segment* segs,
+                                               const int64_t* counts, int64_t num_nodes_cap,
+                                               int64_t num_edges_cap, int32_t* rowptr,
+                                               int32_t* col, uint8_t* ecode, int32_t* rowptr_t,
+                                               int32_t* col_t, uint32_t* nbr, uint32_t* nbr_t,
+                                               int32_t* ecount, int32_t* graph_ptr,
+                                               int32_t* status, void* workspace,
+                                               size_t workspace_bytes, molclr_stream_t stream) {
+  return build_dev(nseg, segs, counts, num_nodes_cap, num_edges_cap, rowptr, col, ecode, rowptr_t,
+                   col_t, nbr, nbr_t, ecount, graph_ptr, status, workspace, workspace_bytes, stream,
+                   true);
+}
diff --git a/molclr_amd/csrc/norm.hip b/molclr_amd/csrc/norm.hip
--- a/molclr_amd/csrc/norm.hip
+++ b/molclr_amd/csrc/norm.hip
@@ -837,19 +837,37 @@
   }
 }
 
-__global__ __launch_bounds__(1024) void k_sum(const float* __restrict__ x, float* __restrict__ out,
-                                              int64_t n) {
+__device__ __forceinline__ float block_sum_ordered(const float* __restrict__ x, int64_t n) {
   __shared__ float ws[16];
   float acc = 0.f;
   for (int64_t i = threadIdx.x; i < n; i += blockDim.x) acc += x[i];
   acc = wave_sum(acc);
   if ((threadIdx.x & 63) == 0) ws[threadIdx.x >> 6] = acc;
   __syncthreads();
-  if (threadIdx.x == 0) {
-    float s = 0.f;
+  float s = 0.f;
+  if (threadIdx.x == 0)
     for (int w = 0; w < (int)(blockDim.x >> 6); ++w) s += ws[w];
-    *out = s;
-  }
+  return s;
+}
+
+__global__ __launch_bounds__(1024) void k_sum(const float* __restrict__ x, float* __restrict__ out,
+                                              int64_t n) {
+  const float s = block_sum_ordered(x, n);
+  if (threadIdx.x == 0) *out = s;
+}
+
+__global__ __launch_bounds__(1024) void k_sum_step_tail(const float* __restrict__ x, int64_t n,
+                                                        float* __restrict__ loss,
+                                                        float* __restrict__ loss_dst,
+                                                        int32_t* __restrict__ step,
+                                                        const int32_t* __restrict__ status_src,
+                                                        int32_t* __restrict__ status_acc) {
+  const float s = block_sum_ordered(x, n);
+  if (threadIdx.x != 0) return;
+  *loss = s;
+  *step += 1;
+  if (loss_dst) *loss_dst = s;
+  if (status_acc) *status_acc |= *status_src;
 }
 
 }
@@ -1458,3 +1476,14 @@
   MOLCLR_LAUNCHED();
   return MOLCLR_OK;
 }
+
+MOLCLR_API int molclr_sum_step_tail(const float* x, int64_t n, float* loss, float* loss_dst,
+                                    int32_t* step, const int32_t* status_src,
+                                    int32_t* status_acc, molclr_stream_t stream) {
+  MOLCLR_REQUIRE(loss && step && (n == 0 || x) && (!status_acc || status_src),
+                 "sum_step_tail: null pointer");
+  hipLaunchKernelGGL(k_sum_step_tail, dim3(1), dim3(1024), 0, molclr::as_stream(stream), x, n, loss,
+                     loss_dst, step, status_src, status_acc);
+  MOLCLR_LAUNCHED();
+  return MOLCLR_OK;
+}
diff --git a/molclr_amd/graph_step.py b/molclr_amd/graph_step.py
--- a/molclr_amd/graph_step.py
+++ b/molclr_amd/graph_step.py
@@ -1,12 +1,16 @@
 from __future__ import annotations
 
 import ctypes
+import os
 from collections import OrderedDict
 
 import torch
 
 from . import _lib, ops
 from .data import DeviceGraph, _num_graphs_of
+
+
+LAUNCH_FOLD = os.environ.get("MOLCLR_LAUNCH_FOLD", "1") != "0"
 
 
 def _round_up(n: int, q: int) -> int:
@@ -45,7 +49,7 @@
         self.graph_ptr = torch.empty(G + 1, **i32)
         self.status = torch.zeros(1, **i32)
         self._ws_bytes = _lib.query("molclr_graph_build_workspace_bytes", N, E)
-        self._ws = torch.empty(self._ws_bytes, dtype=torch.uint8, device=device)
+        self._ws = torch.zeros(self._ws_bytes, dtype=torch.uint8, device=device)
         self._keep = []
 
     def fits(self, views) -> bool:
@@ -79,7 +83,8 @@
         self._keep = keep
 
     def build(self) -> None:
-        _lib.call("molclr_graph_build_dev", self.nseg, ctypes.addressof(self._dst),
+        _lib.call("molclr_graph_build_dev_resident" if LAUNCH_FOLD else "molclr_graph_build_dev",
+                  self.nseg, ctypes.addressof(self._dst),
                   self.counts.data_ptr(), self.num_nodes, self.num_edges,
                   self.rowptr.data_ptr(), self.col.data_ptr(), self.ecode.data_ptr(),
                   self.rowptr_t.data_ptr(), self.col_t.data_ptr(), self.nbr.data_ptr(),
@@ -224,7 +229,11 @@
             if self.reducer is not None:
                 self.reducer.arm()
             _, z = self.model.forward_staged(graph)
-            loss = self.criterion.forward_pair_normalized(z)
+            ops.LOSS_SUM_DEFER = pending = [] if LAUNCH_FOLD and self.group is None else None
+            try:
+                loss = self.criterion.forward_pair_normalized(z)
+            finally:
+                ops.LOSS_SUM_DEFER = None
             loss.backward(self._one)
             if self.reducer is not None:
                 self.reducer.finish()
@@ -232,9 +241,16 @@
                 from .distributed import allreduce_grads
                 allreduce_grads(opt.flat_grad, self.group)
             opt.step(sync_lr=False, tick=False)
-            _lib.call("molclr_step_tail", opt._step_dev.data_ptr(), loss.data_ptr(),
-                      self.loss.data_ptr(), graph.status.data_ptr(), self.status.data_ptr(),
-                      _lib.stream_of(self.device))
+            if pending:
+                (rows, out, n), = pending
+                _lib.call("molclr_sum_step_tail", rows.data_ptr(), n, out.data_ptr(),
+                          self.loss.data_ptr(), opt._step_dev.data_ptr(), graph.status.data_ptr(),
+                          self.status.data_ptr(), _lib.stream_of(self.device))
+            else:
+                _lib.call("molclr_step_tail", opt._step_dev.data_ptr(), loss.data_ptr(),
+                          self.loss.data_ptr(), graph.status.data_ptr(), self.status.data_ptr(),
+                          _lib.stream_of(self.device))
+            del pending
         del loss, z
 
     def _insert(self, ent) -> None:
diff --git a/molclr_amd/ops.py b/molclr_amd/ops.py
--- a/molclr_amd/ops.py
+++ b/molclr_amd/ops.py
@@ -845,7 +845,10 @@
     if _TIMER is not None:
         _TIMER.add("ntxent", 2.0 * n * 2 * B * C)
     loss = torch.empty((), dtype=torch.float32, device=dev)
-    _lib.call("molclr_sum_f32", loss_rows.data_ptr(), loss.data_ptr(), n, st)
+    if LOSS_SUM_DEFER is not None and group is None:
+        LOSS_SUM_DEFER.append((loss_rows, loss, n))
+    else:
+        _lib.call("molclr_sum_f32", loss_rows.data_ptr(), loss.data_ptr(), n, st)
     if group is None:
         lse_cols = lse
     else:
@@ -853,6 +856,9 @@
         lse_cols, loss = mdist.gather_lse_and_sum(lse, loss, group)
     ctx.ntx = (B, C, float(temperature))
     return loss, (cols, gidx, lse_cols, sim)
+
+
+LOSS_SUM_DEFER: list | None = None
 
 
 def _ntxent_rows_backward(ctx, rhat, gloss, cols, gidx, lse_cols, sim):
```

Result: no change. 196,300 molecules/s (median of 5 runs) (+0.2%).
